# seobbro/TTA-depth-completion

Hardware: AMD Instinct MI355X
Metric: TTA frames/sec (fwd+loss+bwd+Adam) at 352x1216 (higher is better)
Workload: dtype mixed: real frames' forward (the scored depth) f32 storage + bf16x3 MFMA arithmetic; no_grad proxy pass and all data gradients bf16 storage + single bf16 MFMA; fp32 accumulate everywhere; loss / Adam / adapted parameters fp32 (include/ptta.h PTTA_DTYPE_MIXED)

## Files before the change

include/ptta.h:

```cpp
#ifndef PTTA_H
#define PTTA_H
#include <stdint.h>
#ifdef __cplusplus
extern "C" {
#endif

typedef struct ptta_ctx* ptta_handle;
typedef void* ptta_stream;

enum { PTTA_BACKBONE_MSG_CHN = 0, PTTA_BACKBONE_NLSPN = 1, PTTA_BACKBONE_COSTDCNET = 2 };
enum { PTTA_DTYPE_F32 = 0, PTTA_DTYPE_MIXED = 1,
       PTTA_MIXED_KEEP_PROXY = 0x100, PTTA_MIXED_KEEP_BACKWARD = 0x200, PTTA_MIXED_KEEP_HEADS = 0x400,
       PTTA_MIXED_BWD_ROUNDED_W = 0x800 };
enum { PTTA_META_1LAYER = 0, PTTA_META_2LAYERS = 1 };
enum { PTTA_NLSPN_LEGACY_OFFSET = 0x100,
       PTTA_NLSPN_SYNCBN_ADAPT = 0x200,
       PTTA_SYNCBN_ADAPT = 0x200 };

typedef struct {
    float lr, beta1, beta2, eps, weight_decay;
    float w_sparse_depth, w_smoothness, w_cos;
    float max_input_depth;
    float max_predict_depth;
} ptta_hparams;
// ... 46 lines not shown
              const float* validity, float* depth_out, float* loss_info_out, ptta_stream s);

int ptta_outlier_removal(const float* sparse_depth, const float* validity, float* sparse_out, float* validity_out,
                         int n, int height, int width, int kernel_size, float threshold, float* scratch, ptta_stream s);

int ptta_eval_metrics(const float* depth, const float* ground_truth, int64_t numel, float min_evaluate_depth,
                      float max_evaluate_depth, void* scratch, float* metrics_out, ptta_stream s);

int ptta_mdconv_forward(const float* input, const float* weight, const float* bias, const float* offset, const float* mask,
                        float* output, int b, int c, int h, int w, int c_out, int kh, int kw, int sh, int sw, int ph, int pw,
                        int dh, int dw, int group, int deformable_group, ptta_stream s);
int ptta_mdconv_backward(const float* input, const float* weight, const float* bias, const float* offset, const float* mask,
                         const float* grad_output, float* grad_input, float* grad_offset, float* grad_mask, float* grad_weight,
                         float* grad_bias, int b, int c, int h, int w, int c_out, int kh, int kw, int sh, int sw, int ph, int pw,
                         int dh, int dw, int group, int deformable_group, ptta_stream s);

int ptta_set_image_norm(ptta_handle h, float divisor, const float* mean, const float* stdv);

int ptta_head_bind(ptta_handle h, const char* name, float* param, float* exp_avg, float* exp_avg_sq);
int ptta_head_set_hparams(ptta_handle h, float lr, float beta1, float beta2, float eps, float weight_decay, float tau,
                          int adam_step, ptta_stream s);
int ptta_head_reload(ptta_handle h, ptta_stream s);
int ptta_head_forward(ptta_handle h, const float* image, const float* sparse_depth, int reverse, float* emb_out, float* ref_out,
                      ptta_stream s);
int ptta_head_backward(ptta_handle h, float* loss_out, ptta_stream s);
int ptta_head_adam_step(ptta_handle h, ptta_stream s);
int ptta_head_step(ptta_handle h, const float* image, const float* sparse_depth, int reverse, float* loss_out, ptta_stream s);
int ptta_head_get_grad(ptta_handle h, const char* name, float* dst, int64_t capacity, int* has_grad_host, ptta_stream s);

enum { PTTA_HEAD_FORM_PLAIN = 0, PTTA_HEAD_FORM_SYNCBN = 1 };
int ptta_head_set_form(ptta_handle h, int form);

int ptta_crop_flip(const float* src, float* dst, int n, int channels, int height, int width, int crop_height, int crop_width,
                   const int32_t* start_y, const int32_t* start_x, const uint8_t* hflip, const uint8_t* vflip, ptta_stream s);

int ptta_rotate(const float* src, float* dst, int n, int channels, int height, int width, const uint8_t* do_rotate, const float* angle_deg,
                int bilinear, ptta_stream s);
int ptta_resize_crop(const float* src, float* dst, int n, int channels, int height, int width, const uint8_t* do_resize,
                     const int32_t* resize_height, const int32_t* resize_width, const int32_t* start_y, const int32_t* start_x,
                     int bilinear, int scale_depth, ptta_stream s);
int ptta_photometric(const float* src, float* dst, int n, int height, int width, const uint8_t* do_brightness, const float* f_brightness,
                     const uint8_t* do_contrast, const float* f_contrast, const uint8_t* do_saturation, const float* f_saturation,
                     double* scratch, ptta_stream s);

int ptta_photometric_full(const float* src, float* dst, int n, int height, int width, const uint8_t* do_brightness, const float* f_brightness,
                          const uint8_t* do_contrast, const float* f_contrast, const uint8_t* do_gamma, const float* f_gamma,
                          const uint8_t* do_hue, const float* f_hue, const uint8_t* do_saturation, const float* f_saturation,
                          double* scratch, ptta_stream s);
int ptta_add_noise(const float* src, const float* noise, float* dst, int n, int channels, int height, int width, const uint8_t* do_noise,
                   float spread, int uniform, ptta_stream s);
int ptta_remove_patches(const float* src, float* dst, int n, int channels, int height, int width, const uint8_t* do_remove,
                        const uint8_t* selected, const int32_t* patch_height, const int32_t* patch_width, ptta_stream s);
int ptta_crop_pad(const float* src, float* dst, int n, int channels, int height, int width, const uint8_t* do_crop_pad,
                  const int32_t* start_y, const int32_t* start_x, const int32_t* end_y, const int32_t* end_x,
                  const int32_t* pad_top, const int32_t* pad_left, int padding_mode, float fill, ptta_stream s);
int ptta_resize_pad(const float* src, float* dst, int n, int channels, int height, int width, const uint8_t* do_resize_pad,
                    const int32_t* resize_height, const int32_t* resize_width, const int32_t* pad_top, const int32_t* pad_left,
                    int bilinear, int padding_mode, float fill, ptta_stream s);

typedef int (*ptta_allreduce_fn)(void* user, double* exchange_buf, long long count, ptta_stream s);
int ptta_set_stat_sync(ptta_handle h, ptta_allreduce_fn fn, void* user, double* exchange_buf, int64_t capacity, int world_size);

int ptta_rccl_unique_id(void* id128_host);
int ptta_rccl_comm_create(const void* id128_host, int rank, int world_size, void** comm_out_host);
int ptta_rccl_comm_destroy(void* comm);
int ptta_rccl_allreduce_mean_f32(void* comm, float* buf, int64_t count, ptta_stream s);
const char* ptta_rccl_last_error(void);
int ptta_set_stat_sync_rccl(ptta_handle h, void* comm, double* exchange_buf, int64_t capacity, int world_size);
int ptta_set_grad_sync_rccl(ptta_handle h, void* comm);

int ptta_set_graph(ptta_handle h, int enable);

int ptta_set_option(ptta_handle h, const char* key, int value);
int ptta_get_option(ptta_handle h, const char* key, int* value_host);

int ptta_profile(ptta_handle h, int enable);
int ptta_profile_read(ptta_handle h, int klass, double* ms_total_host, double* alg_bytes_host, double* macs_host,
                      int64_t* launches_host, ptta_stream s);

int ptta_debug_tensor(ptta_handle h, const char* name, float* dst, int64_t capacity, int64_t* numel_host, ptta_stream s);
int ptta_op_conv32(const float* in_nhwc, const float* weight, const float* bias, float* out_nhwc,
                   int b, int hin, int win, int mode, int relu_in, int in_major, int flip, int dtype, int naive,
                   ptta_stream s);
int ptta_op_gwgrad(const float* x_nhwc, const float* gy_nhwc, float* gw, float* gb, int b, int h, int w, int ci, int co, int impl,
                   int reps, float* us_per_call_host, ptta_stream s);
#define PTTA_GCONV_S1 0
#define PTTA_GCONV_S2 1
#define PTTA_GCONV_T2 2
#define PTTA_GCONV_VERT 1
#define PTTA_GCONV_X1_W2 2
#define PTTA_GCONV_DGRAD 4
int ptta_op_gconv(const float* x0, int c0, int ld0, const float* x1, int c1, int ld1, const float* weight, const float* bias, float* y,
                  int co, int ldy, int b, int hin, int win, int hout, int wout, int k, int geom, int act, int accumulate, int impl,
                  int flags, int six_b, int x1_from_b, int stat_npass, double* stat_host, int* form_host, ptta_stream s);
#define PTTA_GBN_TRAIN 0
#define PTTA_GBN_EVAL 1
#define PTTA_GBN_BACKWARD 2
typedef struct ptta_gbn_view { float* p; int c; int ld; } ptta_gbn_view;
typedef struct ptta_gbn_args {
    int mode, b, h, w, npass, act, act_first, res_relu, acc_gx, acc_gres, world, nblocks_in, repeats;
    float eps, momentum;
    ptta_gbn_view x, res, y, g, gx, gres;
    const float* gamma; const float* beta; const float* part_in;
    float* st; float* rm; float* rv; long long* nbt; float* st_eval; float* dgamma; float* dbeta;
} ptta_gbn_args;
int ptta_op_gbn(const ptta_gbn_args* a, ptta_stream s);
int ptta_op_conv32_chain(const float* in_nhwc, const float* weight, const float* bias, float* buf_a, float* buf_b, const float* aux,
                         int b, int h, int w, int relu_in, int epi_flags, int reps, int replays, float* us_per_launch_host, ptta_stream s);
#define PTTA_ABI_VERSION 2
int ptta_version(void);

#ifdef __cplusplus
}
#endif
#endif
```

tta-depth-completion_amd/csrc/conv32.hip:

```cpp
#include <cstdlib>
#include <cstring>
#include "ptta_common.h"
#include "ptta_kernels.h"

template <typename T>
struct Conv32P {
    const T* in; int in_nb;
    const void* wpack;
    const void* wpack2;
    Epi<T> epi;
    int B, Hin, Win, Hout, Wout;
};

template <typename T> struct Frag;
template <> struct Frag<float> { typedef float4 A; };
template <> struct Frag<bf16_t> { typedef uint4 A; };

__device__ __forceinline__ float4 relu4(float4 v) {
    v.x = fmaxf(v.x, 0.f); v.y = fmaxf(v.y, 0.f); v.z = fmaxf(v.z, 0.f); v.w = fmaxf(v.w, 0.f);
    return v;
}
__device__ __forceinline__ unsigned relu_bf2(unsigned v) {
    unsigned neg = (v >> 15) & 0x00010001u;
    return v & ~(neg * 0xffffu);
// ... 947 lines not shown
    constexpr int STR = F32 ? S2_STR : 48;
    __shared__ __attribute__((aligned(16))) unsigned char lds[NPIX * STR + WL + 16];
    unsigned char* const wl_lds = lds + NPIX * STR;
    const int tid = threadIdx.x, lane = tid & 63;
    const int i = lane & 31, h = lane >> 5;
    const float biasv = epi_bias(p.epi, i);
    const int wave = __builtin_amdgcn_readfirstlane(tid >> 6);
    const int Hin = p.Hin, Win = p.Win, Ho = p.Hout, Wo = p.Wout;
    const int ntx = (Wo + 31) >> 5, nty = (Ho + S2_TH - 1) / S2_TH;
    const long nstages = 2L * p.B * ntx * nty;
    Px<T> v[NIT];
    auto coords = [&](long tile, int& b, int& oy0, int& ox0) {
        long t_ = tile;
        const int ty = (int)(t_ % nty); t_ /= nty;
        const int tx = (int)(t_ % ntx);
        b = (int)(t_ / ntx); oy0 = ty * S2_TH; ox0 = tx << 5;
    };
    auto issue_loads = [&](long stage) {
        int b, oy0, ox0;
        coords(stage >> 1, b, oy0, ox0);
        const T* inb = p.in + (size_t)(b % p.in_nb) * Hin * Win * 32 + 16 * (int)(stage & 1);
#pragma unroll
        for (int it = 0; it < NIT; ++it) {
            const int idx = tid + 256 * it;
            const int g = idx & 1, pix = idx >> 1;
            const int py = pix / S2_PW, px = pix - py * S2_PW;
            const int gy = 2 * oy0 - 1 + py, gx = 2 * ox0 - 1 + px;
            v[it] = px_zero<T>();
            if (pix < NPIX && gy >= 0 && gy < Hin && gx >= 0 && gx < Win) v[it] = px_load(inb + ((size_t)gy * Win + gx) * 32 + 8 * g);
        }
    };
    const long first = 2L * blockIdx.x, sstride = 2L * gridDim.x;
    if (first < nstages) issue_loads(first);
    uint4 wh[9][2];
    load_weights<T, W2>(wh, wl_lds, p.wpack, p.wpack2, tid, lane);
    f32x16 acc;
    bool started = false;
    for (long base = first; base < nstages; base += sstride) {
        int b, oy0, ox0;
        coords(base >> 1, b, oy0, ox0);
#pragma unroll
        for (int q = 0; q < 2; ++q) {
            if (started) lds_barrier();
            started = true;
#pragma unroll
            for (int it = 0; it < NIT; ++it) {
                const int idx = tid + 256 * it;
                const int pix = idx >> 1;
                if (pix < NPIX) px_stage<RELU>(v[it], lds + pix * STR + 16 * (idx & 1), 32);
            }
            {
                const long nxt = q == 0 ? base + 1 : base + sstride;
                if (nxt < nstages) issue_loads(nxt);
            }
            lds_barrier();
            if (q == 0) {
#pragma unroll
                for (int r = 0; r < 16; ++r) acc[r] = 0.f;
            }
            if (oy0 + wave < Ho) {
#pragma unroll
                for (int tap = 0; tap < 9; ++tap) {
                    const int ky = tap / 3, kx = tap % 3;
                    const unsigned char* a = lds + ((2 * wave + ky) * S2_PW + 2 * i + kx) * STR + 16 * h;
                    const bf16x8 ah = __builtin_bit_cast(bf16x8, *(const uint4*)a);
                    const bf16x8 bh = __builtin_bit_cast(bf16x8, wh[tap][q]);
                    if constexpr (F32) {
                        const bf16x8 al = __builtin_bit_cast(bf16x8, *(const uint4*)(a + 32));
                        const bf16x8 bl = __builtin_bit_cast(bf16x8, *(const uint4*)(wl_lds + ((tap * 2 + q) * 64 + lane) * 16));
                        acc = __builtin_amdgcn_mfma_f32_32x32x16_bf16(al, bh, acc, 0, 0, 0);
                        acc = __builtin_amdgcn_mfma_f32_32x32x16_bf16(ah, bl, acc, 0, 0, 0);
                    } else if constexpr (W2) {
                        const bf16x8 bl = __builtin_bit_cast(bf16x8, *(const uint4*)(wl_lds + ((tap * 2 + q) * 64 + lane) * 16));
                        acc = __builtin_amdgcn_mfma_f32_32x32x16_bf16(ah, bl, acc, 0, 0, 0);
                    }
                    acc = __builtin_amdgcn_mfma_f32_32x32x16_bf16(ah, bh, acc, 0, 0, 0);
                }
                if (q == 1) epi_tile<T, false, MASK, ADD>(p.epi, b, oy0 + wave, Ho, Wo, i, acc, ox0, h, Wo, 1, 0, 0.f, 0.f, nullptr, 0, 0, &biasv);
            }
        }
    }
}

template <typename T, int MODE, bool RELU>
__global__ void conv32_naive_kernel(Conv32P<T> p) {
    const long total = (long)p.B * p.Hout * p.Wout * 32;
    const float* wc = (const float*)p.wpack;
    const float sy = up_scale(p.Hout >> 1, p.Hout), sx = up_scale(p.Wout >> 1, p.Wout);
    for (long idx = (long)blockIdx.x * blockDim.x + threadIdx.x; idx < total; idx += (long)gridDim.x * blockDim.x) {
        const int co = (int)(idx & 31);
        long t_ = idx >> 5;
        const int x = (int)(t_ % p.Wout); t_ /= p.Wout;
        const int y = (int)(t_ % p.Hout);
        const int b = (int)(t_ / p.Hout);
        const T* inb = p.in + (size_t)(b % p.in_nb) * p.Hin * p.Win * 32;
        float acc = 0.f;
        for (int tap = 0; tap < 9; ++tap) {
            const int ky = tap / 3, kx = tap % 3;
            int yi, xi;
            if (MODE == CONV_S1) { yi = y + ky - 1; xi = x + kx - 1; }
            else if (MODE == CONV_S2) { yi = 2 * y + ky - 1; xi = 2 * x + kx - 1; }
            else {
                const int ty = y + 1 - ky, tx = x + 1 - kx;
                if ((ty & 1) || (tx & 1)) continue;
                yi = ty >> 1; xi = tx >> 1;
            }
            if (yi < 0 || yi >= p.Hin || xi < 0 || xi >= p.Win) continue;
            const T* src = inb + ((size_t)yi * p.Win + xi) * 32;
            for (int ci = 0; ci < 32; ++ci) {
                float v = ld(src + ci);
                if (RELU) v = fmaxf(v, 0.f);
                acc = fmaf(v, wc[(tap * 32 + ci) * 32 + co], acc);
            }
        }
        Lerp ly = {0, 0, 0.f, 0.f}, lx = {0, 0, 0.f, 0.f};
        if (p.epi.up) { ly = lerp_coef(y, p.Hout >> 1, sy); lx = lerp_coef(x, p.Wout >> 1, sx); }
        epi_store<T>(p.epi, b, y, x, p.Hout, p.Wout, co, acc, ly, lx);
    }
}

__global__ void pack_conv32_kernel(const float* __restrict__ src, float* mf32, bf16_t* mbf16, bf16_t* mlo, float* canon,
                                   int in_major, int flip, int row_stride, int col_off) {
    const int idx = blockIdx.x * blockDim.x + threadIdx.x;
    if (idx >= 9 * 32 * 32) return;
    const int co = idx & 31, ci = (idx >> 5) & 31, tap = idx >> 10;
    const int st = flip ? 8 - tap : tap;
    const float v = in_major ? src[((size_t)ci * row_stride + col_off + co) * 9 + st] : src[((size_t)co * row_stride + col_off + ci) * 9 + st];
    canon[(tap * 32 + ci) * 32 + co] = v;
    {
        const int g = ci >> 3, hh = (ci >> 2) & 1, s = ci & 3;
        mf32[((tap * 4 + g) * 64 + hh * 32 + co) * 4 + s] = v;
    }
    {
        const int kk = ci >> 4, hh = (ci >> 3) & 1, e = ci & 7;
        const bf16_t hi = f2bf(v);
        mbf16[((tap * 2 + kk) * 64 + hh * 32 + co) * 8 + e] = hi;
        mlo[((tap * 2 + kk) * 64 + hh * 32 + co) * 8 + e] = f2bf(v - bf2f(hi));
    }
}

void ptta_pack_conv32(const float* src, const ConvW& w, int in_major, int flip, hipStream_t s, int row_stride, int col_off) {
    hipLaunchKernelGGL(pack_conv32_kernel, dim3(36), dim3(256), 0, s, src, w.mf32, w.mbf16, w.mlo, w.canon, in_major, flip, row_stride, col_off);
}

template <typename T, int MODE, bool RELU>
static void launch_mfma(const Conv32P<T>& p, int flags, int blocks, hipStream_t s) {
#define K_(U, M, A) hipLaunchKernelGGL((conv32_mfma_kernel<T, MODE, RELU, U, M, A>), dim3(blocks), dim3(256), 0, s, p)
    switch (flags) {
        case 0: K_(false, false, false); break; case 1: K_(true, false, false); break;
        case 2: K_(false, true, false); break;  case 3: K_(true, true, false); break;
        case 4: K_(false, false, true); break;  case 5: K_(true, false, true); break;
        case 6: K_(false, true, true); break;   default: K_(true, true, true); break;
    }
#undef K_
}
template <typename T, bool RELU, bool W2 = false>
static void launch_x3(const Conv32P<T>& p, int flags, int blocks, hipStream_t s) {
    const long tiles8 = (long)p.B * ((p.Wout + 31) / 32) * ((p.Hout + X3_TH - 1) / X3_TH);
    if (tiles8 <= 256) {
        const long t4 = (long)p.B * ((p.Wout + 31) / 32) * ((p.Hout + X3S_TH - 1) / X3S_TH);
        const int nb4 = (int)(t4 > 1024 ? 1024 : t4);
#define KS_(U, M, A) hipLaunchKernelGGL((conv32_s1_small_kernel<T, RELU, U, M, A, W2>), dim3(nb4), dim3(256), 0, s, p)
        switch (flags) {
            case 0: KS_(false, false, false); break; case 1: KS_(true, false, false); break;
            case 2: KS_(false, true, false); break;  case 3: KS_(true, true, false); break;
            case 4: KS_(false, false, true); break;  case 5: KS_(true, false, true); break;
// ... 97 lines not shown
            const long tiles = (long)p.B * ((p.Wout + 31) / 32) * ((p.Hout + S2_TH - 1) / S2_TH);
            const int tb = (int)(tiles < kFullChipBlocks ? tiles : kFullChipBlocks);
#define KS2_(R, M, A) hipLaunchKernelGGL((conv32_s2_lds_kernel<T, R, M, A>), dim3(tb), dim3(256), 0, s, p)
            const bool m_ = flags & 2, a_ = flags & 4;
            if (a.relu_in) { if (m_) { if (a_) KS2_(true, true, true); else KS2_(true, true, false); } else { if (a_) KS2_(true, false, true); else KS2_(true, false, false); } }
            else { if (m_) { if (a_) KS2_(false, true, true); else KS2_(false, true, false); } else { if (a_) KS2_(false, false, true); else KS2_(false, false, false); } }
#undef KS2_
            PTTA_CHECK_LAUNCH();
            return 0;
        }
        if constexpr (MODE != CONV_S1) {
            if (a.relu_in) launch_direct_x3<T, MODE, true>(p, flags, (int)blocks, s); else launch_direct_x3<T, MODE, false>(p, flags, (int)blocks, s);
        }
        PTTA_CHECK_LAUNCH();
        return 0;
    }
    if (a.naive) {
        p.wpack = a.w->canon;
        const long total = (long)p.B * p.Hout * p.Wout * 32;
        int blocks = (int)((total + 255) / 256); if (blocks > 8192) blocks = 8192;
        if (a.relu_in) hipLaunchKernelGGL((conv32_naive_kernel<T, MODE, true>), dim3(blocks), dim3(256), 0, s, p);
        else hipLaunchKernelGGL((conv32_naive_kernel<T, MODE, false>), dim3(blocks), dim3(256), 0, s, p);
    } else {
        if (NAR) return -22;
        p.wpack = (const void*)a.w->mf32;
        const int Wt = (MODE == CONV_T2) ? p.Win : p.Wout;
        const long items = (long)p.B * ((Wt + 31) / 32) * (MODE == CONV_T2 ? 2 : 1) * p.Hout;
        long blocks = (items + 3) / 4;
        if (blocks > 512) blocks = 512;
        if constexpr (!NAR) { if (a.relu_in) launch_mfma<T, MODE, true>(p, flags, (int)blocks, s); else launch_mfma<T, MODE, false>(p, flags, (int)blocks, s); }
    }
    PTTA_CHECK_LAUNCH();
    return 0;
}

template <typename T>
static int launch_first_t(const Conv32Args& a, const ConvInArgs& f, void* a_out, int a_nb, bool bwd_form, long tiles, hipStream_t s) {
    Conv32P<T> p;
    p.in = nullptr; p.in_nb = 1; p.wpack = a.w->mbf16; p.wpack2 = (sizeof(T) == 4 || a.w2) ? a.w->mlo : nullptr;
    p.epi.bias = a.bias; p.epi.up = (const T*)a.up; p.epi.up_nb = a.up_nb > 0 ? a.up_nb : 1;
    p.epi.mask = (const T*)a.mask; p.epi.mask_nb = a.mask_nb > 0 ? a.mask_nb : 1; p.epi.add1 = (const T*)a.add1; p.epi.add1_nb = a.add1_nb > 0 ? a.add1_nb : 1; p.epi.add2 = nullptr; p.epi.add2_nb = 1;
    p.epi.out_raw = (T*)a.out_raw; p.epi.out_sum = (T*)a.out_sum;
    p.epi.mask_bits = a.mask_bits; p.epi.bits_out = a.bits_out; p.epi.bits_nb = a.bits_nb; p.epi.bits_sum = 0;
    p.B = a.B; p.Hin = p.Hout = a.Hin; p.Win = p.Wout = a.Win;
    const int blocks = (int)(tiles > kFullChipBlocks ? kFullChipBlocks : tiles);
    FirstP q;
    for (int c = 0; c < 3; ++c) { q.pl[c] = f.pl[c]; if (q.pl[c].nb < 1) q.pl[c].nb = 1; }
    q.zero_from_b = f.zero_from_b; q.w1 = f.wfrag; q.bias1 = f.bias; q.a_out = (float*)a_out; q.a_nb = a_nb;
    q.fmask_nb = f.mask_nb > 0 ? f.mask_nb : 1; q.fmask_bits = f.mask_bits; q.a_bits = f.a_bits;
    if (bwd_form) {
        if constexpr (sizeof(T) == 2) {
            if (a.w2) {
                if (a.out_sum) hipLaunchKernelGGL((conv32_s1_first_kernel<T, 1, false, true, false, true, true, true>), dim3(blocks), dim3(256), 0, s, p, q);
                else hipLaunchKernelGGL((conv32_s1_first_kernel<T, 1, false, true, false, true, false, true>), dim3(blocks), dim3(256), 0, s, p, q);
                PTTA_CHECK_LAUNCH();
                return 0;
            }
        }
        if (a.out_sum) hipLaunchKernelGGL((conv32_s1_first_kernel<T, 1, false, true, false, true, true>), dim3(blocks), dim3(256), 0, s, p, q);
        else hipLaunchKernelGGL((conv32_s1_first_kernel<T, 1, false, true, false, true>), dim3(blocks), dim3(256), 0, s, p, q);
        PTTA_CHECK_LAUNCH();
        return 0;
    }
#define KF_(C) do { if (a.up) hipLaunchKernelGGL((conv32_s1_first_kernel<T, C, true>), dim3(blocks), dim3(256), 0, s, p, q); \
                    else hipLaunchKernelGGL((conv32_s1_first_kernel<T, C, false>), dim3(blocks), dim3(256), 0, s, p, q); } while (0)
    if (f.cin == 1) KF_(1); else if (f.cin == 2) KF_(2); else KF_(3);
#undef KF_
    PTTA_CHECK_LAUNCH();
    return 0;
}
int ptta_launch_conv32_first(const Conv32Args& a, const ConvInArgs& f, void* a_out, int a_nb, hipStream_t s) {
    const bool bwd_form = f.mask != nullptr;
    if (bwd_form && (!f.mask_bits || !a.mask_bits)) return 1;
    if (a.naive || (!a.bf16 && !a.x3) || a.mode != CONV_S1 || a.add2 || f.naive) return 1;
    if ((a.add1 != nullptr) != (a.out_sum != nullptr) || (a.out_sum && !bwd_form)) return 1;
    if (bwd_form ? (a.relu_in || !a.mask || a.up || f.cin != 1) : (!a.relu_in || a.mask != nullptr)) return 1;
    if (f.cin < 1 || f.cin > 3 || f.up || f.add1 || f.B != a.B || f.H != a.Hin || f.W != a.Win) return 1;
    if (a.bf16 && (a_out || f.a_bits)) return 1;
    const long tiles = (long)a.B * ((a.Win + 31) / 32) * ((a.Hin + X3_TH - 1) / X3_TH);
    if (tiles <= 256) return 1;
    return a.bf16 ? launch_first_t<bf16_t>(a, f, a_out, a_nb, bwd_form, tiles, s) : launch_first_t<float>(a, f, a_out, a_nb, bwd_form, tiles, s);
}

int ptta_launch_conv32(const Conv32Args& a, hipStream_t s) {
    if (a.bf16) {
        if (a.mode == CONV_S1) return launch_conv32_t<bf16_t, CONV_S1>(a, s);
        if (a.mode == CONV_S2) return launch_conv32_t<bf16_t, CONV_S2>(a, s);
        return launch_conv32_t<bf16_t, CONV_T2>(a, s);
    }
    if (a.mode == CONV_S1) return launch_conv32_t<float, CONV_S1>(a, s);
    if (a.mode == CONV_S2) return launch_conv32_t<float, CONV_S2>(a, s);
    return launch_conv32_t<float, CONV_T2>(a, s);
}
```

tta-depth-completion_amd/csrc/msgchn_ctx.h:

```cpp
#pragma once
#include <cstdio>
#include <cstdlib>
#include <cstring>
#include <map>
#include <string>
#include <unordered_map>
#include <vector>

#include "../../include/ptta.h"
#include "ptta_common.h"
#include "ptta_kernels.h"
#include "nlspn.h"

#pragma GCC visibility push(hidden)

#define HIPCHK(x) do { hipError_t e_ = (x); if (e_ != hipSuccess) return c->fail(std::string(#x) + ": " + hipGetErrorString(e_), -100 - (int)e_); } while (0)
#define RUN(x) do { int r_ = (x); if (r_ != 0) return c->fail_chain(std::string(#x) + " failed", r_ < 0 ? r_ : -r_); } while (0)

#define NLFWD(call) do { if (c && c->nl) { c->err.clear(); return (call); } } while (0)

struct ImgNorm { int on; float div; float mean[3]; float stdv[3]; };

namespace msgchn {
hipError_t d2d_copy(void* dst, const void* src, size_t bytes, hipStream_t s);
// ... 11 lines not shown
static constexpr unsigned kStepEvent = hipEventDisableTiming | hipEventDisableSystemFence;
struct L32 { ConvW f{}, b{}; float* bias = nullptr; int transposed = 0; };
struct LIn { float *wfrag = nullptr, *wcanon = nullptr, *bias = nullptr, *bw = nullptr; int cin = 1; };
struct LOut { float *w = nullptr, *bias = nullptr, *bfrag = nullptr, *bcanon = nullptr; };
struct Lin { float *W = nullptr, *Wt = nullptr, *bias = nullptr; bf16_t *Whi = nullptr, *Wlo = nullptr, *Wthi = nullptr, *Wtlo = nullptr, *Wil = nullptr, *Wtil = nullptr;
             bf16_t *Wsl = nullptr, *Wtsl = nullptr;
             int N = 0, K = 0; };
struct BNorm { float *gamma = nullptr, *beta = nullptr, *rm = nullptr, *rv = nullptr; long long* nbt = nullptr;
               float *mean = nullptr, *inv = nullptr, *scale = nullptr, *shift = nullptr; };
struct Dbg { const void* p; long numel; int is_act; };

struct PrefixBufs {
    void *c0 = nullptr, *c1 = nullptr, *c2 = nullptr, *c3 = nullptr, *c4 = nullptr, *e1_0a = nullptr, *e1_0 = nullptr, *e1_1a = nullptr;
    void *c0a = nullptr, *c1a = nullptr, *c2a = nullptr, *c3a = nullptr, *c4a = nullptr;
    void *e1_1 = nullptr, *y1 = nullptr, *e1_2a = nullptr, *y2 = nullptr, *t1 = nullptr, *y3 = nullptr, *s1_1 = nullptr, *u1 = nullptr;
    float *dclamp = nullptr, *d12 = nullptr, *d14 = nullptr, *in_image = nullptr, *in_loss_image = nullptr, *in_sparse = nullptr, *in_validity = nullptr;
    bool proxy_valid = false;
};

struct ptta_ctx : PrefixBufs {
    GNet* nl = nullptr;
    int N = 1, H = 0, W = 0, Hp = 0, Wp = 0, pt = 0, pr = 0, dual = 0, Nn = 1;
    int bf16 = 0, naive = 0, es = 4, x3 = 1;
    int mixed = 0;
    int nar_proxy = 0, nar_bwd = 0, nar_heads = 0;
    std::unordered_map<const void*, void*> ntwin;
    void* tw(const void* p) const { auto it = ntwin.find(p); return it == ntwin.end() ? nullptr : it->second; }
    void twin_alloc(const void* p, int nb, int h, int w) { if (nar_proxy && p) ntwin[p] = dalloc((size_t)nb * h * w * 32 * 2); }
    float *dm_f32 = nullptr;
    ptta_hparams hp{};
    std::string err;
    std::vector<void*> allocs;
    std::map<std::string, L32> l32;
    std::map<std::string, LIn> lin_in;
    std::map<std::string, LOut> lout;
    std::map<std::string, Lin> fc;
    std::map<std::string, BNorm> bn;
    std::map<std::string, Dbg> dbg;
    int meta_mode = 0;
    struct Adapted { std::string name; long n = 0; float *p = nullptr, *m = nullptr, *v = nullptr, *g = nullptr; };
    std::vector<Adapted> adapted;
    struct HeadT { bool ready = false; std::vector<Adapted> prm, tgt; bool has_grad[12] = {};
                   float *hyper = nullptr, *tau2 = nullptr, *loss = nullptr, *loss_part = nullptr, *wpart = nullptr, *bpart = nullptr, *dp = nullptr;
                   float *sv_mean = nullptr, *sv_inv = nullptr, *sv_scale = nullptr, *sv_shift = nullptr;
                   int* step = nullptr; unsigned* ticket = nullptr; PttaAdamEntry *tab = nullptr, *etab = nullptr;
                   std::vector<PttaAdamEntry> tab_host, etab_host; int tab_n = 0; long tab_total = 0, etab_total = 0; int tab_mode = -1; bool etab_dirty = true;
                   int reverse = 1; bool fwd_ok = false, bwd_ok = false;
                   float* garena = nullptr; long garena_n = 0;
                   int form = 0; bool stepped = false; } head;
    int skip_dec3 = 0;
    int head_swap = 0;
    float *meta_w = nullptr, *meta_b = nullptr;
    float *gW = nullptr, *gB = nullptr;
    struct Meta2 {
        ConvW w1f[4], w2f[4], w2b[4];
        void *h[4] = {}, *a1[4] = {}, *t = nullptr, *dt = nullptr, *da1 = nullptr, *dh = nullptr;
        float *st1 = nullptr, *st2 = nullptr;
        float *rm1 = nullptr, *rv1 = nullptr, *rm2 = nullptr, *rv2 = nullptr; long long *nbt1 = nullptr, *nbt2 = nullptr;
        float *cs_part = nullptr, *bw = nullptr;
        bool generic = false;
        float *gh = nullptr, *ga1 = nullptr, *gt = nullptr, *gdt = nullptr, *gda1 = nullptr, *gdh = nullptr;
        float *w1c = nullptr, *w2c = nullptr, *w2bc = nullptr;
        bf16_t *w1hi = nullptr, *w1lo = nullptr, *w2hi = nullptr, *w2lo = nullptr, *w2bhi = nullptr, *w2blo = nullptr;
        float *gst1 = nullptr, *gst2 = nullptr, *part1 = nullptr, *part2 = nullptr, *gbw = nullptr, *gpart = nullptr, *wgp = nullptr;
    } m2;
    float* hyper = nullptr;
    float* w3_tmp = nullptr;
    int* step_dev = nullptr; float* stamp_f = nullptr; unsigned long long* stamp_base = nullptr; int stamps = 0;
    void stamp(int i, hipStream_t s) { if (stamps) msgchn::stamp_launch(stamp_f, stamp_base, i, s); }
    PttaAdamEntry* adam_tab = nullptr; unsigned* adam_ticket = nullptr; bool adam_tab_dirty = true;
    std::vector<PttaAdamEntry> adam_host;
    bool fwd_valid = false;
    PttaStatSync stat_sync;
    Lin fused_pp; bool fused_pp_valid = false; int fuse_heads = 1;
    int heads_v2 = 1;
    int thru = 1; bool thru_active = false;
    int adam_in_wgrad = 1; bool adam_fuse_req = false, adam_fused = false;
    int bwd_w2 = 1;
    const float *cnt_sparse = nullptr, *cnt_validity = nullptr;
    struct { const float *image = nullptr, *sparse = nullptr, *validity = nullptr; bool on = false; } loss_report;
    hipEvent_t ev_loss = nullptr;
    hipEvent_t ev_dpart = nullptr;
    int fuse_first = 1, fuse_head_bwd = 1;
    int cos_grad_fused = 1;
    bool cos_in_gemm = false;
    void* w0frag = nullptr; float *hm_part = nullptr, *headP = nullptr; double* head_k12 = nullptr;
    struct ProfClass { std::vector<std::pair<hipEvent_t, hipEvent_t>> ev; size_t used = 0; double bytes = 0, macs = 0; long launches = 0; };
    bool prof_on = false;
    static constexpr int NPROF = 9;
    ProfClass prof[NPROF];
    std::vector<std::pair<int, size_t>> prof_seq;
    int use_graph = 0;
    void* grad_comm = nullptr;
    float* grad_arena = nullptr; long grad_arena_n = 0;
    int pre_sync_graph = -1, pre_sync_aux = -1;
    hipGraphExec_t gexec[4] = {nullptr, nullptr, nullptr, nullptr};
    hipGraph_t graph[4] = {nullptr, nullptr, nullptr, nullptr};
    hipStream_t cap_stream = nullptr;
    struct PreSet : PrefixBufs {
        bool prepared = false, rest_recorded = false;
        uint64_t prep_token = 0;
        uint64_t last_token = 0;
    };
    PreSet pset[2];
    int cur_set = 0, pipe_cur = 0, pipe_last = 0;
    bool pipe_ready = false, pipe_active = false, skip_prefix = false;
    const float *fb_image = nullptr, *fb_sparse = nullptr;
    hipStream_t pre_stream = nullptr;
    hipEvent_t ev_prefix[2] = {nullptr, nullptr}, ev_rest[2] = {nullptr, nullptr}, ev_entry = nullptr;
    hipStream_t pipe_stream = nullptr; bool pipe_stream_set = false;
    hipGraph_t pgraph[2] = {nullptr, nullptr}, rgraph[4][2] = {{nullptr, nullptr}, {nullptr, nullptr}, {nullptr, nullptr}, {nullptr, nullptr}};
    hipGraphExec_t pexec[2] = {nullptr, nullptr}, rexec[4][2] = {{nullptr, nullptr}, {nullptr, nullptr}, {nullptr, nullptr}, {nullptr, nullptr}};
    int use_aux = 1;
    hipStream_t aux_stream = nullptr;
    hipEvent_t ev_fork = nullptr, ev_join = nullptr, ev_real = nullptr;
    hipEvent_t ev_side[4] = {nullptr, nullptr, nullptr, nullptr};
    hipStream_t aux(hipStream_t caller) {
        if (!use_aux) return nullptr;
        if (!aux_stream) {
            if (hipStreamCreateWithFlags(&aux_stream, hipStreamNonBlocking) != hipSuccess) return nullptr;
            if (hipEventCreateWithFlags(&ev_fork, kStepEvent) != hipSuccess ||
                hipEventCreateWithFlags(&ev_join, kStepEvent) != hipSuccess ||
                hipEventCreateWithFlags(&ev_real, kStepEvent) != hipSuccess ||
                hipEventCreateWithFlags(&ev_side[0], kStepEvent) != hipSuccess || hipEventCreateWithFlags(&ev_side[1], kStepEvent) != hipSuccess ||
                hipEventCreateWithFlags(&ev_side[2], kStepEvent) != hipSuccess || hipEventCreateWithFlags(&ev_side[3], kStepEvent) != hipSuccess) { (void)hipStreamDestroy(aux_stream); aux_stream = nullptr; return nullptr; }
        }
        return prof_on ? caller : aux_stream;
    }
    hipEvent_t ev_replay = nullptr;
    void drop_graphs() {
        if (ev_replay) (void)hipEventSynchronize(ev_replay);
        if (pre_stream) (void)hipStreamSynchronize(pre_stream);
        for (int k = 0; k < 4; ++k) {
            if (gexec[k]) { (void)hipGraphExecDestroy(gexec[k]); gexec[k] = nullptr; }
            if (graph[k]) { (void)hipGraphDestroy(graph[k]); graph[k] = nullptr; }
            for (int p = 0; p < 2; ++p) {
                if (rexec[k][p]) { (void)hipGraphExecDestroy(rexec[k][p]); rexec[k][p] = nullptr; }
                if (rgraph[k][p]) { (void)hipGraphDestroy(rgraph[k][p]); rgraph[k][p] = nullptr; }
            }
        }
        for (int p = 0; p < 2; ++p) {
            if (pexec[p]) { (void)hipGraphExecDestroy(pexec[p]); pexec[p] = nullptr; }
            if (pgraph[p]) { (void)hipGraphDestroy(pgraph[p]); pgraph[p] = nullptr; }
            pset[p].prepared = false; pset[p].prep_token = pset[p].last_token = 0;
        }
        fb_image = fb_sparse = nullptr;
    }

    int err_code = 0;
    int fail(const std::string& m, int code) { err = m; err_code = code; return code; }
    int fail_chain(const std::string& m, int code) { err = (err_code == code && !err.empty() && err.size() < 600) ? m + " <- " + err : m; err_code = code; return code; }

    bool oom = false;
    void* dalloc(size_t bytes) {
        void* p = nullptr;
        if (hipMalloc(&p, bytes ? bytes : 16) != hipSuccess) { oom = true; return nullptr; }
        allocs.push_back(p);
        if (hipMemset(p, 0, bytes ? bytes : 16) != hipSuccess) { oom = true; return nullptr; }
        return p;
    }
    float* falloc(size_t n) { return (float*)dalloc(n * sizeof(float)); }
    void* act(const char* name, int nb, int h, int w) {
        void* p = dalloc((size_t)nb * h * w * 32 * es);
        dbg[name] = Dbg{p, (long)nb * h * w * 32, 1};
        if (nar_proxy && nb == 2 * Nn) twin_alloc(p, Nn, h, w);
        return p;
    }
    void* gact(const char* name, int nb, int h, int w) {
        const int e = nar_bwd ? 2 : es;
        void* p = dalloc((size_t)nb * h * w * 32 * e);
        dbg[name] = Dbg{p, (long)nb * h * w * 32, nar_bwd ? 2 : 1};
        return p;
    }
    int mask_bits_on = 1;
    std::unordered_map<const void*, uint32_t*> mbits;
    void mask_plane(const void* map, int nb, int h, int w) {
        if (bf16 || naive) return;
        if (mbits.count(map)) return;
        mbits[map] = (uint32_t*)dalloc((size_t)nb * h * w * sizeof(uint32_t));
    }
    uint32_t* bits_of(const void* map) const {
        if (!map || !mask_bits_on) return nullptr;
        auto it = mbits.find(map);
        return it == mbits.end() ? nullptr : it->second;
    }
    float* map1(const char* name, int nb, int h, int w) {
        float* p = falloc((size_t)nb * h * w);
        dbg[name] = Dbg{p, (long)nb * h * w, 0};
        return p;
    }

    int H2, W2, H4, W4, H8, W8, H16, W16;
    long Rg = 0;
    float *img_pad = nullptr, *sp_pad = nullptr, *zero_plane = nullptr;
    ImgNorm img_norm = ImgNorm{0, 1.f, {0.f, 0.f, 0.f}, {1.f, 1.f, 1.f}};
    float *out1, *p12, *q, *p11, *depth_net, *depth_final, *validity_tmp;
    void *m, *y4, *s0_1, *v1;
    void *e2_0a, *e2_0, *e2_1a, *e2_1, *e2_2a, *z2, *t2, *z3, *s1_2, *u2, *z4, *s0_2, *v2;
    void *e3_0a, *e3_0, *e3_1a, *e3_1, *e3_2a, *feat, *w2, *t3, *s1_3, *u3, *s0_3, *v3;
    float *h1z, *pz, *h2, *emb, *h1, *ref, *gref_buf, *gmask, *bn_part;
    double* hn_msc = nullptr;
    float* hn_rs = nullptr;
    bool cos_rows_done = false;
    bf16_t *emb_n = nullptr, *ref_n = nullptr, *h2_n = nullptr;
    float *bnb_gscale, *bnb_c1, *bnb_c2;
    float *loss_ws, *loss_info, *g_final, *g_net;
    float* loss_info_dst = nullptr;
    void *dv3, *ds0_3, *du3, *ds1_3, *dt3, *dw2, *dfeat_tot, *dz2_up, *de3_2a, *de3_1, *de3_1a, *de3_0, *de3_0a;
    void *up4_t, *up3_t, *dv2, *ds0_2, *dz4, *du2, *ds1_2, *dz3, *dt2, *dz2, *de2_2a, *de2_1, *de2_1a, *de2_0, *de2_0a, *dv1, *dm_total, *g_feat;
    float *dp11, *dq, *dp12, *dout1, *g_feat_f32;
    float* wgrad_part;
};

struct ProfScope {
    ptta_ctx::ProfClass* pc = nullptr; hipStream_t s;
    ProfScope(ptta_ctx* c, int klass, hipStream_t s_, double bytes, double macs, int launches) : s(s_) {
        if (!c->prof_on) return;
        pc = &c->prof[klass];
        if (pc->used == pc->ev.size()) {
            hipEvent_t e0, e1;
            if (hipEventCreate(&e0) != hipSuccess || hipEventCreate(&e1) != hipSuccess) { pc = nullptr; return; }
            pc->ev.push_back({e0, e1});
        }
        pc->bytes += bytes; pc->macs += macs; pc->launches += launches;
        c->prof_seq.push_back({klass, pc->used});
        (void)hipEventRecord(pc->ev[pc->used].first, s);
    }
    ~ProfScope() { if (pc) { (void)hipEventRecord(pc->ev[pc->used].second, s); pc->used++; } }
};
#define REST_(s_, call) do { ProfScope ps_(c, 8, (s_), 0, 0, 1); RUN(call); } while (0)
#define CV(...) RUN(conv32(c, s, __VA_ARGS__))

struct E { const void* up = nullptr; int up_nb = 1; const void* mask = nullptr; int mask_nb = 1;
           const void* add1 = nullptr; int add1_nb = 1; const void* add2 = nullptr; int add2_nb = 1;
           void* raw = nullptr; void* sum = nullptr;
           bool nar = false; };

inline float* st_ptr(float* base, int C, int pass, int kind) { return base + ((size_t)pass * 4 + kind) * C; }

namespace msgchn {
int pad16(int n);
void build_registry(ptta_ctx* c);
void build_workspace(ptta_ctx* c);
int load_weight(ptta_ctx* c, const std::string& name, const void* tensor, const int64_t* shape, int ndim, hipStream_t s);
int conv_in_p(ptta_ctx* c, const ConvInArgs& a_, hipStream_t s);
int conv_out1_p(ptta_ctx* c, const ConvOut1Args& a, hipStream_t s);
int conv32(ptta_ctx* c, hipStream_t s, const std::string& layer, bool bwd, int mode, const void* in, int in_nb,
           int B, int Hin, int Win, bool relu, const E& e);
int conv32w(ptta_ctx* c, hipStream_t s, const ConvW* w, const float* bias, const void* in, int in_nb, int B, int H, int W, const E& e);
int conv32_first_bwd(ptta_ctx* c, hipStream_t s, const std::string& layer, ConvInArgs& f, int B, int H, int W, const E& e);
int to_narrow(ptta_ctx* c, const void* src_f32, void* dst, long n, hipStream_t s);
int to_wide(ptta_ctx* c, const void* src_nar, float* dst, long n, hipStream_t s);
int rgb_encoder(ptta_ctx* c, const float* image, int nb, int boff, int zero_from_b, hipStream_t s);
int ensure_fused_heads(ptta_ctx* c, hipStream_t s);
int ensure_proxy_rgb(ptta_ctx* c, const float* any_image, hipStream_t s);
int enc1_head_fn(ptta_ctx* c, hipStream_t st);
int stage1_independent(ptta_ctx* c, int B2, hipStream_t s);
bool heads_v2_on(const ptta_ctx* c);
int heads_forward(ptta_ctx* c, hipStream_t s, int part = 0);
int push_hparams(ptta_ctx* c, hipStream_t s);
int forward_common(ptta_ctx* c, const float* image, const float* sparse, bool train, hipStream_t s);
const float* final_depth(ptta_ctx* c);
int heads_backward(ptta_ctx* c, const float* gref, hipStream_t s);
int backbone_backward(ptta_ctx* c, const float* g_net, hipStream_t s, bool join_aux);
void pipe_use(ptta_ctx* c, int p);
void pipe_overwritten(ptta_ctx* c, int p);
int pipe_quiesce(ptta_ctx* c);
int ensure_adam_table(ptta_ctx* c, hipStream_t s);
}
#pragma GCC visibility pop
```

tta-depth-completion_amd/csrc/msgchn_forward.hip:

```cpp
#include "msgchn_ctx.h"

using namespace msgchn;

namespace msgchn {

int conv_in_p(ptta_ctx* c, const ConvInArgs& a_, hipStream_t s) {
    ConvInArgs a = a_;
    const double px = (double)a.B * a.H * a.W;
    ProfScope ps(c, 7, s, px * (a.cin * 4 + 32 * (a.bf16 ? 2 : c->es)) + 9.0 * a.cin * 32 * 4, px * 9.0 * a.cin * 32, 1);
    if (!c->mbits.empty()) {
        if (!a.mask_bits) a.mask_bits = c->bits_of(a.mask);
        if (!a.bf16 && !a.a_bits) { a.a_bits = c->bits_of(a.out_raw); a.a_bits_nb = c->Nn; }
    }
    return ptta_launch_conv_in(a, s);
}
int conv_out1_p(ptta_ctx* c, const ConvOut1Args& a, hipStream_t s) {
    const double px = (double)a.B * a.H * a.W;
    ProfScope ps(c, 7, s, px * (32 * (a.bf16 ? 2 : c->es) + 4) + 288 * 4, px * 288.0, 1);
    return ptta_launch_conv_out1(a, s);
}

int conv32(ptta_ctx* c, hipStream_t s, const std::string& layer, bool bwd, int mode, const void* in, int in_nb,
           int B, int Hin, int Win, bool relu, const E& e) {
    auto it = c->l32.find(layer);
    if (it == c->l32.end()) return c->fail("unknown 32->32 layer " + layer, -2);
    Conv32Args a;
    a.in = in; a.in_nb = in_nb; a.w = bwd ? &it->second.b : &it->second.f;
    a.bias = bwd ? nullptr : (layer == "conv1_rgb_meta" ? c->meta_b : it->second.bias);
    a.up = e.up; a.up_nb = e.up_nb; a.mask = e.mask; a.mask_nb = e.mask_nb;
    a.add1 = e.add1; a.add1_nb = e.add1_nb; a.add2 = e.add2; a.add2_nb = e.add2_nb;
    a.out_raw = e.raw; a.out_sum = e.sum;
    const bool nar = e.nar || (bwd && c->nar_bwd);
    const int es_l = nar ? 2 : c->es;
    a.B = B; a.Hin = Hin; a.Win = Win; a.mode = mode; a.relu_in = relu ? 1 : 0; a.bf16 = nar ? 1 : c->bf16; a.naive = c->naive; a.x3 = c->x3;
    a.w2 = (bwd && c->nar_bwd && c->bwd_w2) ? 1 : 0;
    if (!c->mbits.empty()) {
        a.mask_bits = c->bits_of(e.mask);
        if (!bwd && !nar) {
            uint32_t* bs = c->bits_of(e.sum); uint32_t* br = c->bits_of(e.raw);
            if (bs && br) return c->fail("conv32: both outputs of " + layer + " are registered masks", -22);
            if (bs || br) { a.bits_out = bs ? bs : br; a.bits_sum = bs ? 1 : 0; a.bits_nb = c->Nn; }
        }
    }
    const long pin = (long)B * Hin * Win;
    const long pout = mode == CONV_S1 ? pin : (mode == CONV_S2 ? pin / 4 : pin * 4);
    const bool small = (long)Hin * Win <= (long)c->H4 * c->W4 * (mode == CONV_S2 ? 4 : 1);
#ifdef PTTA_EXP_SKIP_PAIRED_S1
    if (mode == CONV_S1 && small && layer.size() > 2 && layer.compare(layer.size() - 2, 2, ".3") == 0 && layer.find("prdct") == std::string::npos) return 0;
#endif
    ProfScope ps(c, (mode == CONV_S1 ? (relu ? 0 : 2) : 4) + (small ? 1 : 0), s, (double)((pin + pout) * 32 + 9216) * es_l,
                 (double)(mode == CONV_T2 ? pin : pout) * 9.0 * 32.0 * 32.0, 1);
    return ptta_launch_conv32(a, s);
}

int conv32w(ptta_ctx* c, hipStream_t s, const ConvW* w, const float* bias, const void* in, int in_nb, int B, int H, int W, const E& e) {
    Conv32Args a;
    a.in = in; a.in_nb = in_nb; a.w = w; a.bias = bias;
    a.add1 = e.add1; a.add1_nb = e.add1_nb; a.out_raw = e.raw; a.out_sum = e.sum;
    a.B = B; a.Hin = H; a.Win = W; a.mode = CONV_S1; a.relu_in = 0; a.bf16 = c->bf16; a.naive = c->naive; a.x3 = c->x3;
    return ptta_launch_conv32(a, s);
}

static int conv32_first(ptta_ctx* c, hipStream_t s, const std::string& layer, ConvInArgs& f, int a_nb, int B, int H, int W, const E& e) {
    auto it = c->l32.find(layer);
    if (it == c->l32.end()) return c->fail("unknown 32->32 layer " + layer, -2);
    const long tiles = (long)B * ((W + 31) / 32) * ((H + 7) / 8);
    const bool nar = e.nar;
    f.bf16 = nar ? 1 : c->bf16;
    if (c->fuse_first >= (f.cin == 3 ? 2 : 1) && !c->bf16 && !c->naive && c->x3 && tiles > 256 && !e.mask && !e.add1 && !e.add2 && !e.sum) {
        Conv32Args a;
        a.in = nullptr; a.in_nb = B; a.w = &it->second.f; a.bias = it->second.bias;
        a.up = e.up; a.up_nb = e.up_nb; a.out_raw = e.raw;
        a.B = B; a.Hin = H; a.Win = W; a.mode = CONV_S1; a.relu_in = 1; a.bf16 = nar ? 1 : 0; a.naive = 0; a.x3 = 1;
        const double px = (double)B * H * W;
        const int es_l = nar ? 2 : c->es;
        ProfScope ps(c, 0, s, (px * f.cin + 9.0 * f.cin * 32) * 4 + (px * 96 + 9216) * es_l, px * 9.0 * (f.cin * 32 + 1024), 1);
        f.a_bits = (a_nb > 0 && !nar) ? c->bits_of(f.out_raw) : nullptr;
        if (!c->mbits.empty() && !nar) { uint32_t* br = c->bits_of(e.raw); if (br) { a.bits_out = br; a.bits_nb = c->Nn; } }
        const int rc = ptta_launch_conv32_first(a, f, (a_nb > 0 && !nar && !f.a_bits) ? f.out_raw : nullptr, a_nb, s);
        return rc == 1 ? c->fail("conv32_first: fused form refused a case its caller accepted", -22) : rc;
    }
    RUN(conv_in_p(c, f, s));
    return conv32(c, s, layer, false, CONV_S1, f.out_raw, B, B, H, W, true, e);
}

int conv32_first_bwd(ptta_ctx* c, hipStream_t s, const std::string& layer, ConvInArgs& f, int B, int H, int W, const E& e) {
    auto it = c->l32.find(layer);
    if (it == c->l32.end()) return c->fail("unknown 32->32 layer " + layer, -2);
    const long tiles = (long)B * ((W + 31) / 32) * ((H + 7) / 8);
    const bool nar = c->nar_bwd != 0;
    f.bf16 = nar ? 1 : c->bf16;
    if (c->fuse_head_bwd && c->bits_of(f.mask) && c->bits_of(e.mask) && c->fuse_first >= 1 && !c->bf16 && !c->naive && c->x3 && tiles > 256 && e.mask && e.raw && (e.add1 != nullptr) == (e.sum != nullptr) && !e.add2 && !e.up) {
        Conv32Args a;
        a.in = nullptr; a.in_nb = B; a.w = &it->second.b; a.bias = nullptr;
        a.mask = e.mask; a.mask_nb = e.mask_nb; a.out_raw = e.raw; a.add1 = e.add1; a.add1_nb = e.add1_nb; a.out_sum = e.sum;
        a.mask_bits = c->bits_of(e.mask); f.mask_bits = c->bits_of(f.mask);
        a.B = B; a.Hin = H; a.Win = W; a.mode = CONV_S1; a.relu_in = 0; a.bf16 = nar ? 1 : 0; a.naive = 0; a.x3 = 1;
        a.w2 = (nar && c->bwd_w2) ? 1 : 0;
        const double px = (double)B * H * W;
        const int es_l = nar ? 2 : c->es;
        ProfScope ps(c, 2, s, (px + 9.0 * 32) * 4 + (px * 96 + 9216) * es_l, px * 9.0 * (32 + 1024), 1);
        const int rc = ptta_launch_conv32_first(a, f, nullptr, 0, s);
        return rc == 1 ? c->fail("conv32_first_bwd: fused form refused a case its caller accepted", -22) : rc;
    }
    RUN(conv_in_p(c, f, s));
    return conv32(c, s, layer, true, CONV_S1, f.out_raw, B, B, H, W, false, e);
}


static int meta_forward(ptta_ctx* c, bool train, int B, hipStream_t s) {
    const int H4 = c->H4, W4 = c->W4, Nn = c->Nn;
    if (c->meta_mode == PTTA_META_1LAYER) {
        E e; e.raw = c->m;
        if (c->nar_proxy && train && B == 2 * Nn) {
            return conv32(c, s, "conv1_rgb_meta", false, CONV_S1, c->c2, Nn, Nn, H4, W4, false, e);
        }
        return conv32(c, s, "conv1_rgb_meta", false, CONV_S1, c->c2, B, B, H4, W4, false, e);
    }
    auto& m2 = c->m2;
    const ptta_ctx::Adapted* A = c->adapted.data();
    const long P = (long)Nn * H4 * W4;
    const int npass = train ? B / Nn : 1;
    if (m2.generic) {
        if (!train && (!m2.rm1 || !m2.rv1 || !m2.rm2 || !m2.rv2)) return c->fail("meta BatchNorm running statistics not loaded", -3);
        GView x; x.p = (float*)c->c2; x.B = B; x.H = H4; x.W = W4; x.C = 32; x.ld = 32;
        GView hv = x; hv.p = m2.gh; hv.C = 128; hv.ld = 128;
        GView av = hv; av.p = m2.ga1;
        GView tv = x; tv.p = m2.gt;
        GView mv = x; mv.p = (float*)c->m;
        const int tiles_pp = ptta_gconv_x3_tiles(B / npass, H4, W4);
        auto finalize = [&](float* part, int C, const float* gamma, const float* beta, float* rm, float* rv, long long* nbt, float* st) -> int {
            if (!train) return ptta_launch_bn_eval_affine(gamma, beta, rm, rv, 1e-5f, st + 2 * C, st + 3 * C, C, s);
            if (ptta_stat_sync(&c->stat_sync, part, tiles_pp, C, npass, s)) return -5;
            const int wmul = c->stat_sync.world > 1 ? c->stat_sync.world : 1;
            for (int pass = 0; pass < npass; ++pass)
// ... 17 lines not shown
        RUN(ptta_launch_gconv_x3(b2, 3, s));
        RUN(finalize(m2.part2, 32, A[5].p, A[6].p, m2.rm2, m2.rv2, m2.nbt2, m2.gst2));
        RUN(ptta_launch_gbn_apply(tv, x, mv, npass, GACT_NONE, m2.gst2, 0, s));
        return 0;
    }
    const int nblk = ptta_chan_stats_blocks();
    for (int g = 0; g < 4; ++g) { E e; e.raw = m2.h[g]; RUN(conv32w(c, s, &m2.w1f[g], nullptr, c->c2, B, B, H4, W4, e)); }
    if (train) {
        for (int pass = 0; pass < npass; ++pass)
            for (int g = 0; g < 4; ++g) {
                RUN(ptta_launch_chan_stats32(m2.h[g], nullptr, c->bf16, pass * P, P, nullptr, nullptr, nullptr, nullptr, -1.f, m2.cs_part, s));
                RUN(ptta_launch_bn_finalize(m2.cs_part, nblk, (int)P, 32, A[1].p + 32 * g, A[2].p + 32 * g, 1e-5f, 0.1f,
                                            m2.rm1 ? m2.rm1 + 32 * g : nullptr, m2.rv1 ? m2.rv1 + 32 * g : nullptr, g == 0 ? m2.nbt1 : nullptr,
                                            st_ptr(m2.st1, 128, pass, 0) + 32 * g, st_ptr(m2.st1, 128, pass, 1) + 32 * g,
                                            st_ptr(m2.st1, 128, pass, 2) + 32 * g, st_ptr(m2.st1, 128, pass, 3) + 32 * g, s));
            }
    } else {
        if (!m2.rm1 || !m2.rv1 || !m2.rm2 || !m2.rv2) return c->fail("meta BatchNorm running statistics not loaded", -3);
        RUN(ptta_launch_bn_eval_affine(A[1].p, A[2].p, m2.rm1, m2.rv1, 1e-5f, st_ptr(m2.st1, 128, 0, 2), st_ptr(m2.st1, 128, 0, 3), 128, s));
    }
    for (int g = 0; g < 4; ++g)
        RUN(ptta_launch_bn_apply32(m2.h[g], nullptr, m2.a1[g], c->bf16, (long)B * H4 * W4, train ? P : (long)B * H4 * W4,
                                   st_ptr(m2.st1, 128, 0, 2) + 32 * g, st_ptr(m2.st1, 128, 0, 3) + 32 * g, 4 * 128, 0.2f, s));
    for (int g = 0; g < 4; ++g) {
        E e;
        if (g == 0) e.raw = m2.t; else { e.add1 = m2.t; e.add1_nb = B; e.sum = m2.t; }
        RUN(conv32w(c, s, &m2.w2f[g], g == 0 ? A[4].p : nullptr, m2.a1[g], B, B, H4, W4, e));
    }
    if (train) {
        for (int pass = 0; pass < npass; ++pass) {
            RUN(ptta_launch_chan_stats32(m2.t, nullptr, c->bf16, pass * P, P, nullptr, nullptr, nullptr, nullptr, -1.f, m2.cs_part, s));
            RUN(ptta_launch_bn_finalize(m2.cs_part, nblk, (int)P, 32, A[5].p, A[6].p, 1e-5f, 0.1f, m2.rm2, m2.rv2, m2.nbt2,
                                        st_ptr(m2.st2, 32, pass, 0), st_ptr(m2.st2, 32, pass, 1), st_ptr(m2.st2, 32, pass, 2), st_ptr(m2.st2, 32, pass, 3), s));
        }
    } else {
        RUN(ptta_launch_bn_eval_affine(A[5].p, A[6].p, m2.rm2, m2.rv2, 1e-5f, st_ptr(m2.st2, 32, 0, 2), st_ptr(m2.st2, 32, 0, 3), 32, s));
    }
    RUN(ptta_launch_bn_apply32(m2.t, c->c2, c->m, c->bf16, (long)B * H4 * W4, train ? P : (long)B * H4 * W4,
                               st_ptr(m2.st2, 32, 0, 2), st_ptr(m2.st2, 32, 0, 3), 4 * 32, -1.f, s));
    return 0;
}


int to_narrow(ptta_ctx* c, const void* src_f32, void* dst, long n, hipStream_t s) {
    if (!src_f32 || !dst) return c->fail("to_narrow: missing narrow twin", -22);
    ProfScope ps_(c, 8, s, 0, 0, 1);
    from_f32_launch((const float*)src_f32, (bf16_t*)dst, n, s);
    return 0;
}
int to_wide(ptta_ctx* c, const void* src_nar, float* dst, long n, hipStream_t s) {
    if (!src_nar || !dst) return c->fail("to_wide: missing operand", -22);
    ProfScope ps_(c, 8, s, 0, 0, 1);
    to_f32_launch((const bf16_t*)src_nar, dst, n, s);
    return 0;
}
static int meta_forward_proxy(ptta_ctx* c, hipStream_t s) {
    const int H4 = c->H4, W4 = c->W4, Nn = c->Nn;
    const long half = (long)Nn * H4 * W4 * 32;
    if (c->meta_mode == PTTA_META_1LAYER) {
        E e; e.raw = c->tw(c->m); e.nar = true;
        return conv32(c, s, "conv1_rgb_meta", false, CONV_S1, c->tw(c->c2), Nn, Nn, H4, W4, false, e);
    }
    return to_narrow(c, (const float*)c->m + half, c->tw(c->m), half, s);
}


int rgb_encoder(ptta_ctx* c, const float* image, int nb, int boff, int zero_from_b, hipStream_t s) {
    const int H1 = c->Hp, W1 = c->Wp, H2 = c->H2, W2 = c->W2, H4 = c->H4, W4 = c->W4, H8 = c->H8, W8 = c->W8, H16 = c->H16, W16 = c->W16;
    auto at = [&](void* base, int h, int w) { return (void*)((char*)base + (size_t)boff * h * w * 32 * c->es); };
    auto e_raw = [](void* raw) { E e; e.raw = raw; return e; };
    {
        const LIn& li = c->lin_in["rgb_encoder.init.0"];
        ConvInArgs a; a.cin = 3; a.zero_from_b = zero_from_b;
        for (int ch = 0; ch < 3; ++ch) {
            a.pl[ch].p = image + (size_t)ch * H1 * W1; a.pl[ch].nb = c->Nn; a.pl[ch].bstride = 3L * H1 * W1;
            if (c->img_norm.on && !c->dual) {
                a.pl[ch].norm = 1; a.pl[ch].div = c->img_norm.div; a.pl[ch].mean = c->img_norm.mean[ch]; a.pl[ch].stdv = c->img_norm.stdv[ch];
            }
        }
        a.wfrag = li.wfrag; a.wcanon = li.wcanon; a.bias = li.bias; a.out_raw = at(c->c0a, H1, W1);
        a.B = nb; a.H = H1; a.W = W1; a.bf16 = c->bf16; a.naive = c->naive;
        RUN(conv32_first(c, s, "rgb_encoder.init.2", a, 0, nb, H1, W1, e_raw(at(c->c0, H1, W1))));
    }
    CV("rgb_encoder.enc1.1", false, CONV_S2, at(c->c0, H1, W1), nb, nb, H1, W1, true, e_raw(at(c->c1a, H2, W2)));
    CV("rgb_encoder.enc1.3", false, CONV_S1, at(c->c1a, H2, W2), nb, nb, H2, W2, true, e_raw(at(c->c1, H2, W2)));
    CV("rgb_encoder.enc2.1", false, CONV_S2, at(c->c1, H2, W2), nb, nb, H2, W2, true, e_raw(at(c->c2a, H4, W4)));
    CV("rgb_encoder.enc2.3", false, CONV_S1, at(c->c2a, H4, W4), nb, nb, H4, W4, true, e_raw(at(c->c2, H4, W4)));
    CV("rgb_encoder.enc3.1", false, CONV_S2, at(c->c2, H4, W4), nb, nb, H4, W4, true, e_raw(at(c->c3a, H8, W8)));
    CV("rgb_encoder.enc3.3", false, CONV_S1, at(c->c3a, H8, W8), nb, nb, H8, W8, true, e_raw(at(c->c3, H8, W8)));
    CV("rgb_encoder.enc4.1", false, CONV_S2, at(c->c3, H8, W8), nb, nb, H8, W8, true, e_raw(at(c->c4a, H16, W16)));
    CV("rgb_encoder.enc4.3", false, CONV_S1, at(c->c4a, H16, W16), nb, nb, H16, W16, true, e_raw(at(c->c4, H16, W16)));
    return 0;
}

int ensure_fused_heads(ptta_ctx* c, hipStream_t s) {
    if (c->fused_pp_valid || !c->fuse_heads) return 0;
    Lin& f = c->fused_pp; const Lin& a = c->fc["proj.3"]; const Lin& b = c->fc["pred.0"];
    fuse_linear_launch(b.W, b.bias, a.W, a.bias, f.W, f.bias, 512, 512, 512, s);
    ptta_split_weight(f.W, f.Whi, f.Wlo, f.Wil, 512L * 512, 512, s);
    ptta_hn_pack_w(f.Whi, f.Wsl, 512, s);
    c->fused_pp_valid = true;
    return 0;
}

int ensure_proxy_rgb(ptta_ctx* c, const float* any_image, hipStream_t s) {
    RUN(ensure_fused_heads(c, s));
    if (c->proxy_valid) return 0;
    RUN(rgb_encoder(c, any_image, c->Nn, c->Nn, 0, s));
    if (c->nar_proxy) {
        const int Nn = c->Nn;
        struct { void* p; int h, w; } maps[4] = {{c->c1, c->H2, c->W2}, {c->c2, c->H4, c->W4}, {c->c3, c->H8, c->W8}, {c->c4, c->H16, c->W16}};
        for (auto& m_ : maps) {
            const long half = (long)Nn * m_.h * m_.w * 32;
            RUN(to_narrow(c, (const float*)m_.p + half, c->tw(m_.p), half, s));
        }
    }
    c->proxy_valid = true;
    return 0;
}

int enc1_head_fn(ptta_ctx* c, hipStream_t st) {
    const int Nn = c->Nn, H4 = c->H4, W4 = c->W4;
    const LIn& li = c->lin_in["depth_encoder1.init.0"];
    ConvInArgs a; a.cin = 1; a.pl[0].p = c->d14; a.pl[0].nb = Nn; a.pl[0].bstride = (long)H4 * W4;
    a.wfrag = li.wfrag; a.wcanon = li.wcanon; a.bias = li.bias; a.out_raw = c->e1_0a;
    a.B = Nn; a.H = H4; a.W = W4; a.bf16 = c->bf16; a.naive = c->naive;
    RUN(conv_in_p(c, a, st));
    { E e; e.raw = c->e1_0; RUN(conv32(c, st, "depth_encoder1.init.2", false, CONV_S1, c->e1_0a, Nn, Nn, H4, W4, true, e)); }
    { E e; e.raw = c->e1_1a; RUN(conv32(c, st, "depth_encoder1.enc1.1", false, CONV_S2, c->e1_0, Nn, Nn, H4, W4, true, e)); }
    return 0;
}

int stage1_independent(ptta_ctx* c, int B2, hipStream_t s) {
    const int Nn = c->Nn, H4 = c->H4, W4 = c->W4, H8 = c->H8, W8 = c->W8, H16 = c->H16, W16 = c->W16;
    const bool two = c->nar_proxy && B2 == 2 * Nn;
    const int Bf = two ? Nn : B2;
    { E e; e.raw = c->e1_1; e.sum = c->y1; e.add1 = c->c3; e.add1_nb = B2;
      RUN(conv32(c, s, "depth_encoder1.enc1.3", false, CONV_S1, c->e1_1a, Nn, Bf, H8, W8, true, e)); }
    { E e; e.raw = c->e1_2a; RUN(conv32(c, s, "depth_encoder1.enc2.1", false, CONV_S2, c->e1_1, B2, Nn, H8, W8, true, e)); }
    { E e; e.sum = c->y2; e.add1 = c->c4; e.add1_nb = B2;
      RUN(conv32(c, s, "depth_encoder1.enc2.3", false, CONV_S1, c->e1_2a, Nn, Bf, H16, W16, true, e)); }
    { E e; e.raw = c->t1; RUN(conv32(c, s, "depth_decoder1.dec2.1", false, CONV_T2, c->y2, B2, Bf, H16, W16, true, e)); }
    { E e; e.raw = c->y3; e.sum = c->s1_1; e.add1 = c->y1; e.add1_nb = B2;
      RUN(conv32(c, s, "depth_decoder1.dec2.3", false, CONV_S1, c->t1, B2, Bf, H8, W8, true, e)); }
    { E e; e.raw = c->u1; RUN(conv32(c, s, "depth_decoder1.dec1.1", false, CONV_T2, c->s1_1, B2, Bf, H8, W8, true, e)); }
    if (!two) return 0;
    RUN(to_narrow(c, c->e1_0, c->tw(c->e1_0), (long)Nn * H4 * W4 * 32, s));
    RUN(to_narrow(c, c->e1_1a, c->tw(c->e1_1a), (long)Nn * H8 * W8 * 32, s));
    RUN(to_narrow(c, c->e1_2a, c->tw(c->e1_2a), (long)Nn * H16 * W16 * 32, s));
    { E e; e.nar = true; e.sum = c->tw(c->y1); e.add1 = c->tw(c->c3); e.add1_nb = Nn;
      RUN(conv32(c, s, "depth_encoder1.enc1.3", false, CONV_S1, c->tw(c->e1_1a), Nn, Nn, H8, W8, true, e)); }
    { E e; e.nar = true; e.sum = c->tw(c->y2); e.add1 = c->tw(c->c4); e.add1_nb = Nn;
      RUN(conv32(c, s, "depth_encoder1.enc2.3", false, CONV_S1, c->tw(c->e1_2a), Nn, Nn, H16, W16, true, e)); }
    { E e; e.nar = true; e.raw = c->tw(c->t1); RUN(conv32(c, s, "depth_decoder1.dec2.1", false, CONV_T2, c->tw(c->y2), Nn, Nn, H16, W16, true, e)); }
    { E e; e.nar = true; e.raw = c->tw(c->y3); e.sum = c->tw(c->s1_1); e.add1 = c->tw(c->y1); e.add1_nb = Nn;
      RUN(conv32(c, s, "depth_decoder1.dec2.3", false, CONV_S1, c->tw(c->t1), Nn, Nn, H8, W8, true, e)); }
    { E e; e.nar = true; e.raw = c->tw(c->u1); RUN(conv32(c, s, "depth_decoder1.dec1.1", false, CONV_T2, c->tw(c->s1_1), Nn, Nn, H8, W8, true, e)); }
    return 0;
}

static int backbone(ptta_ctx* c, const float* image, bool train, hipStream_t s) {
    hipStream_t s2 = train ? c->aux(s) : nullptr;
    const int Nn = c->Nn, B2 = train ? 2 * Nn : Nn;
    const bool two = train && c->nar_proxy;
    const int H1 = c->Hp, W1 = c->Wp, H2 = c->H2, W2 = c->W2, H4 = c->H4, W4 = c->W4, H8 = c->H8, W8 = c->W8, H16 = c->H16, W16 = c->W16;
    auto e_raw = [](void* raw) { E e; e.raw = raw; return e; };
    if (!c->skip_prefix) RUN(rgb_encoder(c, image, Nn, 0, Nn, s));
    RUN(meta_forward(c, train, B2, s));
    if (!c->skip_prefix) { RUN(enc1_head_fn(c, s)); RUN(stage1_independent(c, B2, s)); }

    auto region = [&](hipStream_t st, int b0, int Bl, bool nar) -> int {
        auto A = [&](void* p_, int h, int w) -> void* { return nar ? c->tw(p_) : (void*)((char*)p_ + (size_t)b0 * h * w * 32 * c->es); };
        auto P1 = [&](float* p_, int h, int w) { return p_ + (size_t)b0 * h * w; };
        auto raw = [&](void* r) { E e; e.raw = r; e.nar = nar; return e; };
        const void* e1_0 = nar ? c->tw(c->e1_0) : c->e1_0;
#define CR(...) RUN(conv32(c, st, __VA_ARGS__))
        { E e; e.nar = nar; e.raw = A(c->y4, H4, W4); e.sum = A(c->s0_1, H4, W4); e.add1 = e1_0; e.add1_nb = Nn; e.add2 = A(c->m, H4, W4); e.add2_nb = Bl;
          CR("depth_decoder1.dec1.3", false, CONV_S1, A(c->u1, H4, W4), Bl, Bl, H4, W4, true, e); }
        CR("depth_decoder1.prdct.1", false, CONV_S1, A(c->s0_1, H4, W4), Bl, Bl, H4, W4, true, raw(A(c->v1, H4, W4)));
        {
            const LOut& lo = c->lout["depth_decoder1.prdct.3"];
            ConvOut1Args a; a.in = A(c->v1, H4, W4); a.in_nb = Bl; a.w = lo.w; a.bias = lo.bias; a.out = P1(c->out1, H4, W4);
            a.B = Bl; a.H = H4; a.W = W4; a.relu_in = 1; a.bf16 = nar ? 1 : c->bf16;
            RUN(conv_out1_p(c, a, st));
        }
        REST_(st, ptta_launch_up2_1ch(P1(c->out1, H4, W4), P1(c->p12, H2, W2), Bl, H4, W4, st));
        {
            const LIn& li = c->lin_in["depth_encoder2.init.0"];
            ConvInArgs a; a.cin = 2;
            a.pl[0].p = c->d12; a.pl[0].nb = Nn; a.pl[0].bstride = (long)H2 * W2;
            a.pl[1].p = P1(c->p12, H2, W2); a.pl[1].nb = Bl; a.pl[1].bstride = (long)H2 * W2;
            a.wfrag = li.wfrag; a.wcanon = li.wcanon; a.bias = li.bias; a.out_raw = A(c->e2_0a, H2, W2);
            a.B = Bl; a.H = H2; a.W = W2; a.bf16 = c->bf16; a.naive = c->naive;
            E e; e.nar = nar; e.raw = A(c->e2_0, H2, W2); e.up = A(c->y4, H4, W4); e.up_nb = Bl;
            RUN(conv32_first(c, st, "depth_encoder2.init.2", a, (b0 == 0 && !nar) ? Nn : 0, Bl, H2, W2, e));
        }
        CR("depth_encoder2.enc1.1", false, CONV_S2, A(c->e2_0, H2, W2), Bl, Bl, H2, W2, true, raw(A(c->e2_1a, H4, W4)));
        { E e; e.nar = nar; e.raw = A(c->e2_1, H4, W4); e.up = A(c->y3, H8, W8); e.up_nb = Bl; CR("depth_encoder2.enc1.3", false, CONV_S1, A(c->e2_1a, H4, W4), Bl, Bl, H4, W4, true, e); }
        CR("depth_encoder2.enc2.1", false, CONV_S2, A(c->e2_1, H4, W4), Bl, Bl, H4, W4, true, raw(A(c->e2_2a, H8, W8)));
        { E e; e.nar = nar; e.sum = A(c->z2, H8, W8); e.up = A(c->y2, H16, W16); e.up_nb = Bl; e.add1 = A(c->c3, H8, W8); e.add1_nb = Bl;
          CR("depth_encoder2.enc2.3", false, CONV_S1, A(c->e2_2a, H8, W8), Bl, Bl, H8, W8, true, e); }
        CR("depth_decoder2.dec2.1", false, CONV_T2, A(c->z2, H8, W8), Bl, Bl, H8, W8, true, raw(A(c->t2, H4, W4)));
        { E e; e.nar = nar; e.raw = A(c->z3, H4, W4); e.sum = A(c->s1_2, H4, W4); e.add1 = A(c->e2_1, H4, W4); e.add1_nb = Bl; e.add2 = A(c->m, H4, W4); e.add2_nb = Bl;
          CR("depth_decoder2.dec2.3", false, CONV_S1, A(c->t2, H4, W4), Bl, Bl, H4, W4, true, e); }
        CR("depth_decoder2.dec1.1", false, CONV_T2, A(c->s1_2, H4, W4), Bl, Bl, H4, W4, true, raw(A(c->u2, H2, W2)));
        { E e; e.nar = nar; e.raw = A(c->z4, H2, W2); e.sum = A(c->s0_2, H2, W2); e.add1 = A(c->e2_0, H2, W2); e.add1_nb = Bl; e.add2 = A(c->c1, H2, W2); e.add2_nb = Bl;
          CR("depth_decoder2.dec1.3", false, CONV_S1, A(c->u2, H2, W2), Bl, Bl, H2, W2, true, e); }
        CR("depth_decoder2.prdct.1", false, CONV_S1, A(c->s0_2, H2, W2), Bl, Bl, H2, W2, true, raw(A(c->v2, H2, W2)));
        {
            const LOut& lo = c->lout["depth_decoder2.prdct.3"];
            ConvOut1Args a; a.in = A(c->v2, H2, W2); a.in_nb = Bl; a.w = lo.w; a.bias = lo.bias; a.add = P1(c->p12, H2, W2); a.add_nb = Bl; a.out = P1(c->q, H2, W2);
            a.B = Bl; a.H = H2; a.W = W2; a.relu_in = 1; a.bf16 = nar ? 1 : c->bf16;
            RUN(conv_out1_p(c, a, st));
        }
        REST_(st, ptta_launch_up2_1ch(P1(c->q, H2, W2), P1(c->p11, H1, W1), Bl, H2, W2, st));
        {
            const LIn& li = c->lin_in["depth_encoder3.init.0"];
            ConvInArgs a; a.cin = 2;
            a.pl[0].p = c->dclamp; a.pl[0].nb = Nn; a.pl[0].bstride = (long)H1 * W1;
            a.pl[1].p = P1(c->p11, H1, W1); a.pl[1].nb = Bl; a.pl[1].bstride = (long)H1 * W1;
            a.wfrag = li.wfrag; a.wcanon = li.wcanon; a.bias = li.bias; a.out_raw = A(c->e3_0a, H1, W1);
            a.B = Bl; a.H = H1; a.W = W1; a.bf16 = c->bf16; a.naive = c->naive;
            E e; e.nar = nar; e.raw = A(c->e3_0, H1, W1); e.up = A(c->z4, H2, W2); e.up_nb = Bl;
            RUN(conv32_first(c, st, "depth_encoder3.init.2", a, (b0 == 0 && !nar) ? Nn : 0, Bl, H1, W1, e));
        }
        CR("depth_encoder3.enc1.1", false, CONV_S2, A(c->e3_0, H1, W1), Bl, Bl, H1, W1, true, raw(A(c->e3_1a, H2, W2)));
        { E e; e.nar = nar; e.raw = A(c->e3_1, H2, W2); e.up = A(c->z3, H4, W4); e.up_nb = Bl; CR("depth_encoder3.enc1.3", false, CONV_S1, A(c->e3_1a, H2, W2), Bl, Bl, H2, W2, true, e); }
        CR("depth_encoder3.enc2.1", false, CONV_S2, A(c->e3_1, H2, W2), Bl, Bl, H2, W2, true, raw(A(c->e3_2a, H4, W4)));
        { E e; e.nar = nar; e.raw = A(c->feat, H4, W4); e.up = A(c->z2, H8, W8); e.up_nb = Bl; e.add1 = A(c->m, H4, W4); e.add1_nb = Bl;
          if (!nar) e.sum = A(c->w2, H4, W4); else e.add1 = nullptr;
          CR("depth_encoder3.enc2.3", false, CONV_S1, A(c->e3_2a, H4, W4), Bl, Bl, H4, W4, true, e); }
#undef CR
        return 0;
    };
    if (two) {
        hipStream_t sp = s2 ? s2 : s;
        if (s2) { HIPCHK(hipEventRecord(c->ev_fork, s)); HIPCHK(hipStreamWaitEvent(s2, c->ev_fork, 0)); }
        c->stamp(3, sp);
        if (s2 && c->thru_active && c->cnt_sparse) REST_(s2, ptta_launch_loss_valid_count(c->cnt_sparse, c->cnt_validity, c->N, c->H, c->W, c->loss_ws, s2));
        RUN(meta_forward_proxy(c, sp));
        c->stamp(1, s);
        RUN(region(s, 0, Nn, false));
        c->stamp(2, s);
        RUN(region(sp, Nn, Nn, true));
        c->stamp(4, sp);
        const bool hn = c->nar_heads && heads_v2_on(c);
        if (!hn) RUN(to_wide(c, c->tw(c->feat), (float*)c->feat + (size_t)c->Rg * 32, c->Rg * 32, sp));
        if (s2) {
            if (hn) RUN(heads_forward(c, s2, 1));
            c->stamp(5, s2);
            HIPCHK(hipEventRecord(c->ev_real, s)); HIPCHK(hipStreamWaitEvent(s2, c->ev_real, 0));
            RUN(heads_forward(c, s2, hn ? 2 : 0));
            c->stamp(6, s2);
            HIPCHK(hipEventRecord(c->ev_join, s2));
        }
    } else {
        RUN(region(s, 0, B2, false));
        if (train && s2) {
            HIPCHK(hipEventRecord(c->ev_fork, s)); HIPCHK(hipStreamWaitEvent(s2, c->ev_fork, 0));
            if (c->thru_active && c->cnt_sparse) REST_(s2, ptta_launch_loss_valid_count(c->cnt_sparse, c->cnt_validity, c->N, c->H, c->W, c->loss_ws, s2));
            RUN(heads_forward(c, s2));
            HIPCHK(hipEventRecord(c->ev_join, s2));
        }
    }
    if (!c->skip_dec3) {
    CV("depth_decoder3.dec2.1", false, CONV_T2, c->w2, B2, Nn, H4, W4, true, e_raw(c->t3));
    { E e; e.sum = c->s1_3; e.add1 = c->e3_1; e.add1_nb = B2; e.add2 = c->c1; e.add2_nb = B2;
      CV("depth_decoder3.dec2.3", false, CONV_S1, c->t3, Nn, Nn, H2, W2, true, e); }
    CV("depth_decoder3.dec1.1", false, CONV_T2, c->s1_3, Nn, Nn, H2, W2, true, e_raw(c->u3));
    { E e; e.sum = c->s0_3; e.add1 = c->e3_0; e.add1_nb = B2; e.add2 = c->c0; e.add2_nb = B2;
      CV("depth_decoder3.dec1.3", false, CONV_S1, c->u3, Nn, Nn, H1, W1, true, e); }
    CV("depth_decoder3.prdct.1", false, CONV_S1, c->s0_3, Nn, Nn, H1, W1, true, e_raw(c->v3));
    {
        const LOut& lo = c->lout["depth_decoder3.prdct.3"];
        ConvOut1Args a; a.in = c->v3; a.in_nb = Nn; a.w = lo.w; a.bias = lo.bias; a.add = c->p11; a.add_nb = B2; a.out = c->depth_net;
        a.B = Nn; a.H = H1; a.W = W1; a.relu_in = 1; a.bf16 = c->bf16;
        RUN(conv_out1_p(c, a, s));
    }
    }
    c->stamp(7, s);
    if (train) {
        if (s2) { if (!c->thru_active) HIPCHK(hipStreamWaitEvent(s, c->ev_join, 0)); }
        else RUN(heads_forward(c, s));
    }
    return 0;
}

bool heads_v2_on(const ptta_ctx* c) {
    return c->heads_v2 && c->fuse_heads && c->fused_pp_valid && c->x3 && !c->bf16 && !c->naive && !c->skip_dec3 && !c->head_swap;
}

static int mlp_forward(ptta_ctx* c, const std::string& name, const void* A, int a_bf16, int K, float* hidden, float* out, hipStream_t s) {
    const Lin& l0 = c->fc[name + ".0"]; const Lin& l3 = c->fc[name + ".3"]; BNorm& bn = c->bn[name + ".1"];
    const int R = (int)c->Rg;
    GemmArgs g; g.A = A; g.a_bf16 = a_bf16; g.W = l0.W; g.bias = l0.bias; g.C = hidden; g.R = R; g.K = K; g.N = 512; g.epi = 1; g.part = c->bn_part;
    g.x3 = c->x3; g.Whi = l0.Whi; g.Wlo = l0.Wlo; g.Wil = l0.Wil;
    RUN(ptta_launch_gemm(g, s));
    RUN(ptta_stat_sync(&c->stat_sync, c->bn_part, ptta_gemm_part_blocks(g), 512, 1, s));
    RUN(ptta_launch_bn_finalize(c->bn_part, ptta_gemm_part_blocks(g), R * (c->stat_sync.world > 1 ? c->stat_sync.world : 1), 512, bn.gamma, bn.beta, 1e-5f, 0.1f, bn.rm, bn.rv, bn.nbt,
                                bn.mean, bn.inv, bn.scale, bn.shift, s));
    GemmArgs g2; g2.A = hidden; g2.W = l3.W; g2.bias = l3.bias; g2.C = out; g2.R = R; g2.K = 512; g2.N = 512; g2.pro = 1;
    g2.pscale = bn.scale; g2.pshift = bn.shift;
    g2.x3 = c->x3; g2.Whi = l3.Whi; g2.Wlo = l3.Wlo; g2.Wil = l3.Wil;
    RUN(ptta_launch_gemm(g2, s));
    return 0;
}

int heads_forward(ptta_ctx* c, hipStream_t s, int part) {
    if (part != 1) c->cos_rows_done = false;
    const double esh = (c->nar_heads && heads_v2_on(c)) ? 2.0 : 4.0;
    ProfScope ps_(c, 6, s, (double)c->Rg * 2 * 32 * 4 + ((double)c->Rg * (2 * 512 + 4 * 1024) + 2 * 16384.0 + 4 * 262144.0) * esh,
                  (double)c->Rg * (2 * 16384.0 + 4 * 262144.0), heads_v2_on(c) ? 7 : 8);
    const size_t half = (size_t)c->Rg * 32 * c->es;
    const void* feat_zero = (const char*)c->feat + half;
    if (c->nar_heads && heads_v2_on(c)) {
        const Lin& l0 = c->fc["proj.0"]; const Lin& lf = c->fused_pp; const Lin& lp3 = c->fc["pred.3"]; const Lin& l3 = c->fc["proj.3"];
        BNorm& b1 = c->bn["proj.1"]; BNorm& b2 = c->bn["pred.1"];
        const long R = c->Rg; const int Rw = (int)R * (c->stat_sync.world > 1 ? c->stat_sync.world : 1);
        const int nbh = 2, nb = ptta_hn_row_blocks(R);
        float* part_real = c->hm_part; float* part_zero = c->hm_part + (size_t)nbh * 2 * 512;
        double* msc_real = c->hn_msc; double* msc_zero = c->hn_msc + (size_t)ptta_hn_moment_scratch(R);
        HnBnOut bo1; bo1.gamma = b1.gamma; bo1.beta = b1.beta; bo1.rm = b1.rm; bo1.rv = b1.rv; bo1.nbt = b1.nbt;
        bo1.mean = b1.mean; bo1.inv = b1.inv; bo1.scale = b1.scale; bo1.shift = b1.shift;
        auto gemm_h = [&](const void* x, int x_bf16, const Lin& w, bf16_t* out, int epi) {
            HnGemmArgs g; g.pro = 3; g.epi = epi; g.X = x; g.x_bf16 = x_bf16; g.W0 = l0.Whi; g.b0 = l0.bias; g.pscale = b1.scale; g.pshift = b1.shift;
            g.W = w.Wsl; g.bias = w.bias; g.C = out; g.part = c->bn_part; g.R = R;
            return g;
        };
        if (part != 2) {
            const void* xz = c->nar_proxy ? (const void*)c->tw(c->feat) : (const void*)((const float*)c->feat + (size_t)R * 32);
            if (!c->stat_sync.on()) RUN(ptta_launch_hn_moments(xz, c->nar_proxy ? 1 : 0, R, 1, l0.W, l0.bias, msc_zero, nullptr, &bo1, s));
            else {
            RUN(ptta_launch_hn_moments(xz, c->nar_proxy ? 1 : 0, R, 1, l0.W, l0.bias, msc_zero, part_zero, nullptr, s));
            RUN(ptta_stat_sync(&c->stat_sync, part_zero, nbh, 512, 1, s));
            RUN(ptta_launch_bn_finalize(part_zero, nbh, Rw, 512, b1.gamma, b1.beta, 1e-5f, 0.1f, b1.rm, b1.rv, b1.nbt, b1.mean, b1.inv, b1.scale, b1.shift, s));
            }
            if (c->nar_proxy) RUN(ptta_launch_hn_gemm(gemm_h(c->tw(c->feat), 1, lf, c->h2_n, 1), s));
            else RUN(ptta_launch_hn_gemm(gemm_h((const float*)c->feat + (size_t)R * 32, 0, lf, c->h2_n, 1), s));
            RUN(ptta_stat_sync(&c->stat_sync, c->bn_part, nb, 512, 1, s));
            RUN(ptta_launch_bn_finalize(c->bn_part, nb, Rw, 512, b2.gamma, b2.beta, 1e-5f, 0.1f, b2.rm, b2.rv, b2.nbt, b2.mean, b2.inv, b2.scale, b2.shift, s));
            HnGemmArgs g3; g3.pro = 1; g3.epi = 2; g3.A = c->h2_n; g3.pscale = b2.scale; g3.pshift = b2.shift; g3.W = lp3.Wsl; g3.bias = lp3.bias; g3.C = c->emb_n; g3.R = R;
            g3.rs = c->hn_rs;
            RUN(ptta_launch_hn_gemm(g3, s));
        }
        if (part != 1) {
            if (!c->stat_sync.on()) RUN(ptta_launch_hn_moments(c->feat, 0, R, 1, l0.W, l0.bias, msc_real, nullptr, &bo1, s));
            else {
            RUN(ptta_launch_hn_moments(c->feat, 0, R, 1, l0.W, l0.bias, msc_real, part_real, nullptr, s));
            RUN(ptta_stat_sync(&c->stat_sync, part_real, nbh, 512, 1, s));
            RUN(ptta_launch_bn_finalize(part_real, nbh, Rw, 512, b1.gamma, b1.beta, 1e-5f, 0.1f, b1.rm, b1.rv, b1.nbt, b1.mean, b1.inv, b1.scale, b1.shift, s));
            }
            HnGemmArgs gr = gemm_h(c->feat, 0, l3, c->ref_n, 5);
            gr.E = c->emb_n; gr.rs = c->hn_rs; gr.rowstats_out = c->loss_ws + ptta_loss_ws_rows_off(c->N);
            gr.cpart = c->loss_ws + ptta_loss_ws_cos_off(c->N, c->Rg); gr.cpart_n = ptta_loss_cos_blocks(c->Rg);
// ... 131 lines not shown
```

tta-depth-completion_amd/csrc/ptta_api.hip:

```cpp
#include "msgchn_ctx.h"

using namespace msgchn;

int msgchn::ensure_adam_table(ptta_ctx* c, hipStream_t s) {
    if (!c->adam_tab_dirty) return 0;
    for (auto& ad : c->adapted) if (!ad.p || !ad.m || !ad.v) return 0;
    c->adam_host.resize(c->adapted.size());
    long off = 0;
    for (size_t k = 0; k < c->adapted.size(); ++k) { auto& ad = c->adapted[k]; c->adam_host[k] = PttaAdamEntry{ad.p, ad.m, ad.v, ad.g, ad.n, off}; off += ad.n; }
    HIPCHK(hipMemcpyAsync(c->adam_tab, c->adam_host.data(), c->adam_host.size() * sizeof(PttaAdamEntry), hipMemcpyHostToDevice, s));
    c->adam_tab_dirty = false;
    return 0;
}

extern "C" {

int ptta_version(void) { return PTTA_ABI_VERSION; }

const char* ptta_last_error(ptta_handle h) { return h ? (h->nl && h->err.empty() ? h->nl->err.c_str() : h->err.c_str()) : "null handle"; }

static int wrap_gnet(ptta_handle* out, GNet* e, int rc, int gmix, int n, int height, int width, const ptta_hparams* hp) {
    if (!e) return rc ? rc : -12;
    e->mixed = e->naive ? 0 : gmix;
    ptta_ctx* c = new ptta_ctx();
// ... 280 lines not shown
int ptta_adam_step(ptta_handle c, const float* gw, const float* gb, ptta_stream s_) {
    if (c && c->nl) return (gw || gb) ? c->fail("explicit gradients are an MSG_CHN 1layer convenience", -22) : c->nl->adam_step((hipStream_t)s_);

    if (!c) return -1;
    for (auto& ad : c->adapted) if (!ad.p || !ad.m || !ad.v) return c->fail("Adam state of " + ad.name + " not bound", -3);
    if ((gw || gb) && c->meta_mode != PTTA_META_1LAYER) return c->fail("explicit gradients are a 1layer convenience; use the internal ones", -22);
    hipStream_t s = (hipStream_t)s_;
    if (!gw && !gb) {
        RUN(ensure_adam_table(c, s));
        long total = 0; for (auto& ad : c->adapted) total += ad.n;
        REST_(s, ptta_launch_adam_multi(c->adam_tab, (int)c->adapted.size(), total, c->hyper, c->step_dev, c->adam_ticket, s));
        return 0;
    }
    RUN(ptta_launch_step_inc(c->step_dev, s));
    for (size_t k = 0; k < c->adapted.size(); ++k) {
        auto& ad = c->adapted[k];
        const float* g = ad.g;
        if (c->meta_mode == PTTA_META_1LAYER) { if (k == 0 && gw) g = gw; if (k == 1 && gb) g = gb; }
        RUN(ptta_launch_adam(ad.p, ad.m, ad.v, g, ad.n, c->hyper, c->step_dev, s));
    }
    return 0;
}

int ptta_set_image_norm(ptta_handle c, float divisor, const float* mean, const float* stdv) {
    NLFWD(c->nl->set_image_norm(divisor, mean, stdv));

    if (!c) return -1;
    if (!(divisor > 0.f)) return c->fail("ptta_set_image_norm: divisor must be positive", -22);
    ImgNorm nm = ImgNorm{0, divisor, {0.f, 0.f, 0.f}, {1.f, 1.f, 1.f}};
    for (int k = 0; k < 3; ++k) {
        if (mean) nm.mean[k] = mean[k];
        if (stdv) { if (!(stdv[k] > 0.f)) return c->fail("ptta_set_image_norm: std must be positive", -22); nm.stdv[k] = stdv[k]; }
    }
    nm.on = !(divisor == 1.f && nm.mean[0] == 0.f && nm.mean[1] == 0.f && nm.mean[2] == 0.f && nm.stdv[0] == 1.f &&
              nm.stdv[1] == 1.f && nm.stdv[2] == 1.f);
    c->img_norm = nm;
    c->drop_graphs();
    return 0;
}

static int set_stat_sync(ptta_ctx* c, const PttaStatSync& sy, bool on, bool keeps_graph) {
    if (c->nl) { c->err.clear(); c->nl->drop_graphs(); c->nl->stat_sync = sy; return 0; }
    if (on && c->meta_mode == PTTA_META_2LAYERS && !c->m2.generic) return c->fail("SyncBatchNorm needs the default arithmetic for the 2layers meta layer", -38);
    c->stat_sync = sy;
    c->drop_graphs();
    if (on) {
        if (c->pre_sync_graph < 0) { c->pre_sync_graph = c->use_graph; c->pre_sync_aux = c->use_aux; }
        else if (keeps_graph) c->use_graph = c->pre_sync_graph;
        if (!keeps_graph) c->use_graph = 0;
        c->use_aux = 0;
    } else if (c->pre_sync_graph >= 0) {
        c->use_graph = c->pre_sync_graph; c->use_aux = c->pre_sync_aux; c->pre_sync_graph = c->pre_sync_aux = -1;
    }
    return 0;
}

int ptta_set_stat_sync(ptta_handle c, ptta_allreduce_fn fn, void* user, double* exchange_buf, int64_t capacity, int world_size) {
    if (!c || world_size < 1 || (world_size > 1 && (!fn || !exchange_buf || capacity < 2 * 1024))) return -22;
    PttaStatSync sy; sy.fn = (ptta_allreduce_cb)fn; sy.user = user; sy.buf = exchange_buf; sy.cap = (long)capacity; sy.world = world_size;
    return set_stat_sync(c, sy, world_size > 1, false);
}

int ptta_set_stat_sync_rccl(ptta_handle c, void* comm, double* exchange_buf, int64_t capacity, int world_size) {
    if (!c || world_size < 1 || (comm && (!exchange_buf || capacity < 2 * 1024))) return -22;
    PttaStatSync sy; sy.comm = comm; sy.buf = exchange_buf; sy.cap = (long)capacity; sy.world = world_size;
    return set_stat_sync(c, sy, comm != nullptr, true);
}

int ptta_set_grad_sync_rccl(ptta_handle c, void* comm) {
    if (!c) return -1;
    if (c->nl) { c->nl->drop_graphs(); c->nl->grad_comm = comm; return 0; }
    c->grad_comm = comm;
    c->drop_graphs();
    return 0;
}

struct Option { const char* key; int ptta_ctx::*member; int hi; bool mixed_free; };
static const Option kOptions[] = {
    {"aux_stream", &ptta_ctx::use_aux, 1, true},        {"thru", &ptta_ctx::thru, 1, true},
    {"adam_in_wgrad", &ptta_ctx::adam_in_wgrad, 1, true}, {"bwd_w2", &ptta_ctx::bwd_w2, 1, true},
    {"fuse_first", &ptta_ctx::fuse_first, 2, false},    {"fuse_head_bwd", &ptta_ctx::fuse_head_bwd, 1, false},
    {"fuse_heads", &ptta_ctx::fuse_heads, 1, false},    {"heads_v2", &ptta_ctx::heads_v2, 1, false},
    {"cos_in_gemm", &ptta_ctx::cos_grad_fused, 1, false}, {"mask_bits", &ptta_ctx::mask_bits_on, 1, false},
    {"stamps", &ptta_ctx::stamps, 1, true},
};
static const Option* find_option(const std::string& k) {
    for (const Option& o : kOptions) if (k == o.key) return &o;
    return nullptr;
}
int ptta_set_option(ptta_handle c, const char* key, int value) {
    if (!c || !key) return -1;
    const std::string k(key);
    if (k == "graph") return ptta_set_graph(c, value);
    if (c->nl) return -38;
    const Option* o = find_option(k);
    if (!o) return c->fail("ptta_set_option: unknown key '" + k + "'", -22);
    int* f = &(c->*(o->member));
    if (value < 0 || value > o->hi) return c->fail("ptta_set_option: value out of range for '" + k + "'", -22);
    if (c->mixed && !o->mixed_free && value != 1)
        return c->fail("ptta_set_option: the mixed mode is defined on the default kernels ('" + k + "' stays 1)", -38);
    if (k == "aux_stream" && c->pre_sync_graph >= 0) { c->pre_sync_aux = value; return 0; }
    if (*f == value) return 0;
    RUN(pipe_quiesce(c));
    c->drop_graphs();
    *f = value;
    return 0;
}

int ptta_get_option(ptta_handle c, const char* key, int* value) {
    if (!c || !key || !value) return -1;
    const std::string k(key);
    if (k == "pipelined_active") { *value = !(c->nl || c->prof_on || c->dual || c->stat_sync.on() || c->grad_comm || c->naive || c->bf16); return 0; }
    if (k == "thru_active") { *value = c->nl ? 0 : (c->thru && c->cos_grad_fused && heads_v2_on(c) && c->use_aux); return 0; }
    if (c->nl) { if (k != "graph") return -38; *value = c->nl->use_graph; return 0; }
    if (k == "graph") { *value = c->use_graph; return 0; }
    const Option* o = find_option(k);
    if (!o) return -22;
    *value = c->*(o->member);
    return 0;
}

int ptta_set_graph(ptta_handle c, int enable) {
    if (c && c->nl) { c->nl->use_graph = enable ? 1 : 0; if (!enable) c->nl->drop_graphs(); return 0; }

    if (!c) return -1;
    if (enable && c->stat_sync.on() && !c->stat_sync.comm) return c->fail("graph replay is not available with SyncBatchNorm exchange (ptta_set_stat_sync)", -38);
    c->use_graph = enable ? 1 : 0;
    if (!enable) c->drop_graphs();
    return 0;
}

int ptta_profile(ptta_handle c, int enable) {
    if (c && c->nl) return c->fail("not available for the NLSPN / CostDCNet backbones: use ptta_step / ptta_forward_*", -38);

    if (!c) return -1;
    c->prof_on = enable != 0;
    for (auto& pc : c->prof) { pc.used = 0; pc.bytes = 0; pc.macs = 0; pc.launches = 0; }
    c->prof_seq.clear();
    return 0;
}

int ptta_profile_read(ptta_handle c, int klass, double* ms_total, double* alg_bytes, double* macs, int64_t* launches, ptta_stream s_) {
    if (c && c->nl) return c->fail("not available for the NLSPN / CostDCNet backbones: use ptta_step / ptta_forward_*", -38);

    if (!c || klass < 0 || klass >= ptta_ctx::NPROF) return -1;
    HIPCHK(hipStreamSynchronize((hipStream_t)s_));
    ptta_ctx::ProfClass& pc = c->prof[klass];
    double ms = 0;
    for (size_t k = 0; k < pc.used; ++k) {
        float t = 0.f;
        HIPCHK(hipEventElapsedTime(&t, pc.ev[k].first, pc.ev[k].second));
        ms += t;
    }
    if (ms_total) *ms_total = ms;
    if (alg_bytes) *alg_bytes = pc.bytes;
    if (macs) *macs = pc.macs;
    if (launches) *launches = (int64_t)pc.launches;
    return 0;
}

int ptta_debug_tensor(ptta_handle c, const char* name, float* dst, int64_t capacity, int64_t* numel_host, ptta_stream s_) {
    NLFWD(c->nl->debug_tensor(name, dst, capacity, numel_host, (hipStream_t)s_));

    if (!c || !name) return -1;
    if (std::string(name) == "prof_seq") {
        HIPCHK(hipStreamSynchronize((hipStream_t)s_));
        const int64_t n = 2 * (int64_t)c->prof_seq.size();
// ... 28 lines not shown
```

tta-depth-completion_amd/csrc/ptta_kernels.h:

```cpp
#pragma once
#include <hip/hip_runtime.h>
#include <cstdlib>
#include <cstring>
#include "ptta_common.h"

struct PttaCreateEnv { int naive = 0, exact = 0, graph = -1; };
inline PttaCreateEnv ptta_create_env() {
    PttaCreateEnv e;
    const char* v = getenv("PTTA_CONV_IMPL"); e.naive = (v && strcmp(v, "naive") == 0) ? 1 : 0;
    v = getenv("PTTA_ARITH"); e.exact = (v && strcmp(v, "exact") == 0) ? 1 : 0;
    v = getenv("PTTA_GRAPH"); e.graph = (v && (strcmp(v, "0") == 0 || strcmp(v, "1") == 0)) ? (v[0] - '0') : -1;
    return e;
}

struct ConvW {
    float* mf32;
    bf16_t* mbf16;
    bf16_t* mlo;
    float* canon;
};
struct Conv32Args {
    const void* in = nullptr; int in_nb = 1;
    const ConvW* w = nullptr;
    const float* bias = nullptr;
    const void* up = nullptr; int up_nb = 1;
    const void* mask = nullptr; int mask_nb = 1;
    const void* add1 = nullptr; int add1_nb = 1;
    const void* add2 = nullptr; int add2_nb = 1;
    void* out_raw = nullptr; void* out_sum = nullptr;
    int B = 1, Hin = 0, Win = 0;
    int mode = CONV_S1; int relu_in = 0; int bf16 = 0; int naive = 0;
    int x3 = 0;
    int w2 = 0;
    const uint32_t* mask_bits = nullptr;
    uint32_t* bits_out = nullptr; int bits_nb = 0; int bits_sum = 0;
};
void ptta_pack_conv32(const float* src, const ConvW& w, int in_major, int flip, hipStream_t s, int row_stride = 32, int col_off = 0);
int ptta_launch_conv32(const Conv32Args& a, hipStream_t s);
int ptta_launch_conv32_loop(const Conv32Args& a, void* buf_a, void* buf_b, int reps, unsigned* ctr, unsigned* base_io, int* err, int variant, hipStream_t s);

struct Plane { const float* p = nullptr; int nb = 1; long bstride = 0;
               int norm = 0; float div = 1.f, mean = 0.f, stdv = 1.f; };
struct ConvInArgs {
    Plane pl[3]; int cin = 1; int zero_from_b = 1 << 30;
    const float* wfrag = nullptr;
    const float* wcanon = nullptr;
    const float* bias = nullptr;
    const void* up = nullptr; int up_nb = 1;
    const void* mask = nullptr; int mask_nb = 1;
    const void* add1 = nullptr; int add1_nb = 1;
    void* out_raw = nullptr; void* out_sum = nullptr;
    int B = 1, H = 0, W = 0; int bf16 = 0; int naive = 0;
    const uint32_t* mask_bits = nullptr; uint32_t* a_bits = nullptr;
    int a_bits_nb = 0;
};
void ptta_pack_conv_in(const float* src, int cin_total, int cin_first, int cin, int transpose_flip,
                       float* wfrag, float* wcanon, hipStream_t s);
int ptta_launch_conv_in(const ConvInArgs& a, hipStream_t s);
int ptta_launch_conv32_first(const Conv32Args& a, const ConvInArgs& f, void* a_out, int a_nb, hipStream_t s);

struct ConvOut1Args {
    const void* in = nullptr; int in_nb = 1;
    const float* w = nullptr;
    const float* bias = nullptr;
    const float* add = nullptr; int add_nb = 1;
    float* out = nullptr;
    int B = 1, H = 0, W = 0; int relu_in = 0; int bf16 = 0;
};
void ptta_pack_conv_out1(const float* src, int src_cin_total, int src_cin_index, int from_conv_in, float* w, hipStream_t s);
int ptta_launch_conv_out1(const ConvOut1Args& a, hipStream_t s);

int ptta_launch_prep(const float* sparse, float max_input_depth, float* dclamp, float* d12, float* d14,
                     int N, int H, int W, hipStream_t s);
int ptta_launch_up2_1ch(const float* in, float* out, int B, int Hin, int Win, hipStream_t s);
int ptta_launch_up2T_1ch(const float* gout, float* gin, int B, int Hin, int Win, hipStream_t s);
int ptta_launch_up2T_32(const void* gout, const void* add, void* gin, int B, int Hin, int Win, int bf16, hipStream_t s);

int ptta_launch_outlier_removal(const float* sparse, const float* validity, float* sparse_out, float* validity_out,
                                int N, int H, int W, int ksize, float threshold, float* scratch, hipStream_t s);

typedef int (*ptta_allreduce_cb)(void* user, double* dev_buf, long long count, void* stream);
int ptta_rccl_sum_f64(void* comm, double* buf, long long count, hipStream_t s);
struct PttaStatSync {
    ptta_allreduce_cb fn = nullptr; void* user = nullptr;
    void* comm = nullptr;
    double* buf = nullptr; long cap = 0; int world = 1;
    bool on() const { return (fn || comm) && (world > 1 || comm); }
    int exchange(long long count, hipStream_t s) const {
        if (comm) return ptta_rccl_sum_f64(comm, buf, count, s);
        const int rc = fn(user, buf, count, (void*)s);
        return rc ? (rc < 0 ? rc : -rc) : 0;
    }
};
int ptta_stat_sync(const PttaStatSync* sy, float* part, int nblocks, int C, int npass, hipStream_t s);
int ptta_grad_mean_sync(const PttaStatSync* sy, float* g, long n, hipStream_t s);

struct GemmArgs {
    const void* A = nullptr; int a_bf16 = 0;
    const float* A2 = nullptr;
    const float* W = nullptr;
    const float* bias = nullptr;
    float* C = nullptr;
    int R = 0, K = 0, N = 0;
    int pro = 0;
    const float* pscale = nullptr; const float* pshift = nullptr;
    const float* pmean = nullptr; const float* pinv = nullptr;
    const float* pc1 = nullptr; const float* pc2 = nullptr;
    int epi = 0;
    const float* eH = nullptr;
    const float* escale = nullptr; const float* eshift = nullptr; const float* emean = nullptr; const float* einv = nullptr;
    float* part = nullptr;
    int x3 = 0; const bf16_t* Whi = nullptr; const bf16_t* Wlo = nullptr;
    const bf16_t* Wil = nullptr;
    const float* X = nullptr;
    const void* W0frag = nullptr;
    const float* b0 = nullptr;
    const bf16_t* W0hi = nullptr; const bf16_t* W0lo = nullptr;
    const bf16_t* W0thi = nullptr; const bf16_t* W0tlo = nullptr;
    float* P = nullptr;
    const float* Bref = nullptr; const float* rowstats = nullptr; const float* coef = nullptr;
};
// ... 195 lines not shown
```

tta-depth-completion_amd/csrc/ptta_ops.hip:

```cpp
#include "msgchn_ctx.h"
#include "gnet.h"

using namespace msgchn;

namespace {
struct ScratchConvW {
    ConvW w{};
    bool ok;
    ScratchConvW() {
        ok = hipMalloc((void**)&w.mf32, 9 * 4 * 64 * 4 * 4) == hipSuccess && hipMalloc((void**)&w.mbf16, 9 * 2 * 64 * 8 * 2) == hipSuccess &&
             hipMalloc((void**)&w.canon, 9216 * 4) == hipSuccess && hipMalloc((void**)&w.mlo, 9 * 2 * 64 * 8 * 2) == hipSuccess;
    }
    ~ScratchConvW() { (void)hipFree(w.mf32); (void)hipFree(w.mbf16); (void)hipFree(w.mlo); (void)hipFree(w.canon); }
    ScratchConvW(const ScratchConvW&) = delete;
    ScratchConvW& operator=(const ScratchConvW&) = delete;
};

__global__ void op_scale_f64_kernel(double* buf, long long n, double f) {
    for (long long i = (long long)blockIdx.x * blockDim.x + threadIdx.x; i < n; i += (long long)gridDim.x * blockDim.x) buf[i] *= f;
}
int op_gbn_exchange(void* user, double* buf, long long count, void* stream) {
    long long blocks = (count + 255) / 256; if (blocks > 1024) blocks = 1024; if (blocks < 1) blocks = 1;
    hipLaunchKernelGGL(op_scale_f64_kernel, dim3((int)blocks), dim3(256), 0, (hipStream_t)stream, buf, count, (double)*(const int*)user);
    return hipGetLastError() == hipSuccess ? 0 : -5;
}
}

extern "C" {

int ptta_outlier_removal(const float* sparse, const float* validity, float* sparse_out, float* validity_out, int n, int height,
                         int width, int kernel_size, float threshold, float* scratch, ptta_stream s) {
    if (!sparse || !validity || !sparse_out || !validity_out || !scratch || n < 1 || height < 1 || width < 1 || kernel_size < 1 ||
        (kernel_size & 1) == 0) return -22;
    return ptta_launch_outlier_removal(sparse, validity, sparse_out, validity_out, n, height, width, kernel_size, threshold, scratch,
                                       (hipStream_t)s);
}

int ptta_eval_metrics(const float* depth, const float* ground_truth, int64_t numel, float min_evaluate_depth, float max_evaluate_depth,
                      void* scratch, float* metrics_out, ptta_stream s) {
    if (!depth || !ground_truth || !scratch || !metrics_out || numel < 1) return -22;
    return ptta_launch_eval_metrics(depth, ground_truth, numel, min_evaluate_depth, max_evaluate_depth, (double*)scratch, metrics_out,
                                    (hipStream_t)s);
}

static void dcn_args(DcnArgs& a, const float* input, const float* weight, const float* bias, const float* offset, const float* mask,
                     int b, int c, int h, int w, int c_out, int kh, int kw, int sh, int sw, int ph, int pw, int dh, int dw, int group, int dg) {
    a.in = input; a.weight = weight; a.bias = bias; a.offset = offset; a.mask = mask;
    a.B = b; a.C = c; a.H = h; a.W = w; a.Co = c_out; a.kh = kh; a.kw = kw; a.sh = sh; a.sw = sw; a.ph = ph; a.pw = pw;
    a.dh = dh; a.dw = dw; a.group = group; a.dg = dg;
}

int ptta_mdconv_forward(const float* input, const float* weight, const float* bias, const float* offset, const float* mask, float* output,
                        int b, int c, int h, int w, int c_out, int kh, int kw, int sh, int sw, int ph, int pw, int dh, int dw,
                        int group, int deformable_group, ptta_stream s) {
    if (!input || !weight || !offset || !mask || !output) return -22;
    DcnArgs a; dcn_args(a, input, weight, bias, offset, mask, b, c, h, w, c_out, kh, kw, sh, sw, ph, pw, dh, dw, group, deformable_group);
    a.out = output;
    return ptta_launch_dcn_forward(a, (hipStream_t)s);
}

int ptta_mdconv_backward(const float* input, const float* weight, const float* bias, const float* offset, const float* mask,
                         const float* grad_output, float* grad_input, float* grad_offset, float* grad_mask, float* grad_weight,
                         float* grad_bias, int b, int c, int h, int w, int c_out, int kh, int kw, int sh, int sw, int ph, int pw,
                         int dh, int dw, int group, int deformable_group, ptta_stream s) {
    if (!input || !weight || !offset || !mask || !grad_output) return -22;
    DcnArgs a; dcn_args(a, input, weight, bias, offset, mask, b, c, h, w, c_out, kh, kw, sh, sw, ph, pw, dh, dw, group, deformable_group);
    a.gout = grad_output; a.gin = grad_input; a.goff = grad_offset; a.gmask = grad_mask; a.gweight = grad_weight; a.gbias = grad_bias;
    return ptta_launch_dcn_backward(a, (hipStream_t)s);
}

int ptta_op_conv32(const float* in, const float* weight, const float* bias, float* out, int b, int hin, int win, int mode,
                   int relu_in, int in_major, int flip, int dtype, int naive, ptta_stream s_) {
    hipStream_t s = (hipStream_t)s_;
    ScratchConvW sw; ConvW& w = sw.w;
    void *tin = nullptr, *tout = nullptr;
    const int ho = mode == CONV_S1 ? hin : (mode == CONV_S2 ? hin / 2 : hin * 2), wo = mode == CONV_S1 ? win : (mode == CONV_S2 ? win / 2 : win * 2);
    const long nin = (long)b * hin * win * 32, nout = (long)b * ho * wo * 32;
    int rc = 0;
    if (!sw.ok || hipMalloc(&tin, nin * 2) != hipSuccess || hipMalloc(&tout, nout * 2) != hipSuccess) rc = -12;
    if (rc == 0) {
        ptta_pack_conv32(weight, w, in_major, flip, s);
        Conv32Args a; a.w = &w; a.bias = bias; a.B = b; a.Hin = hin; a.Win = win; a.mode = mode; a.relu_in = relu_in; a.naive = naive & 1; a.x3 = (naive >> 1) & 1;
        if (dtype != PTTA_DTYPE_F32) {
            from_f32_launch(in, (bf16_t*)tin, nin, s);
            a.in = tin; a.in_nb = b; a.out_raw = tout; a.bf16 = 1;
            rc = ptta_launch_conv32(a, s);
            to_f32_launch((const bf16_t*)tout, out, nout, s);
        } else {
            a.in = in; a.in_nb = b; a.out_raw = out; a.bf16 = 0;
            rc = ptta_launch_conv32(a, s);
        }
        (void)hipStreamSynchronize(s);
    }
    (void)hipFree(tin); (void)hipFree(tout);
    return rc;
}

int ptta_op_gwgrad(const float* x, const float* gy, float* gw, float* gb, int b, int h, int w, int ci, int co, int impl, int reps,
                   float* us_per_call_host, ptta_stream s_) {
    hipStream_t s = (hipStream_t)s_;
    if (!x || !gy || !gw || b < 1 || h < 1 || w < 1 || ci < 1 || co < 1 || ci > 256 || co > 256 || impl < 0 || impl > 2 || reps < 0 ||
        (reps > 0 && !us_per_call_host)) return -22;
    GView xv, gv;
    xv.p = (float*)x; xv.B = b; xv.H = h; xv.W = w; xv.C = ci; xv.ld = ci;
    gv.p = (float*)gy; gv.B = b; gv.H = h; gv.W = w; gv.C = co; gv.ld = co;
    const long P = (long)b * h * w;
    const size_t nm = (size_t)ptta_gwgrad_mfma_part_floats(P, ci, co), nn = (size_t)ptta_gwgrad_slabs(P) * (9 * ci * co + co);
    float* part = nullptr;
    if (hipMalloc((void**)&part, (impl == 2 ? nn : nm) * 4) != hipSuccess) return -12;
    auto run = [&]() {
        return impl == 0 ? ptta_launch_gwgrad_mfma(xv, gv, part, gw, gb, s)
                         : (impl == 1 ? ptta_launch_gwgrad_f32mfma(xv, gv, part, gw, gb, s) : ptta_launch_gwgrad(xv, gv, part, gw, gb, s));
    };
    int rc = run();
    if (!rc && reps > 0) {
        hipEvent_t e0 = nullptr, e1 = nullptr;
        if (hipEventCreate(&e0) != hipSuccess || hipEventCreate(&e1) != hipSuccess) rc = -5;
        if (!rc) {
            (void)hipEventRecord(e0, s);
            for (int r = 0; r < reps && !rc; ++r) rc = run();
            (void)hipEventRecord(e1, s);
            (void)hipEventSynchronize(e1);
            float ms = 0.f; (void)hipEventElapsedTime(&ms, e0, e1);
            *us_per_call_host = 1e3f * ms / (float)reps;
        }
        if (e0) (void)hipEventDestroy(e0);
        if (e1) (void)hipEventDestroy(e1);
    }
    if (hipStreamSynchronize(s) != hipSuccess && !rc) rc = -5;
    (void)hipFree(part);
    return rc;
}

int ptta_op_gconv(const float* x0, int c0, int ld0, const float* x1, int c1, int ld1, const float* weight, const float* bias, float* y, int co,
                  int ldy, int b, int hin, int win, int hout, int wout, int k, int geom, int act, int accumulate, int impl, int flags,
                  int six_b, int x1_from_b, int stat_npass, double* stat_host, int* form_host, ptta_stream s_) {
    hipStream_t s = (hipStream_t)s_;
    const bool vert = flags & PTTA_GCONV_VERT, dgrad = flags & PTTA_GCONV_DGRAD;
    if (!x0 || !weight || !y || b < 1 || hin < 1 || win < 1 || hout < 1 || wout < 1 || c0 < 1 || c1 < 0 || co < 1 || ld0 < c0 || ldy < co ||
        (c1 > 0) != (x1 != nullptr) || (c1 > 0 && ld1 < c1) || (k != 1 && k != 3) || geom < PTTA_GCONV_S1 || geom > PTTA_GCONV_T2 ||
        act < GACT_NONE || act > GACT_SIGMOID || impl < 0 || impl > 1 || (flags & ~7) || six_b < 0 || six_b > b || x1_from_b < 0 ||
        stat_npass < 0 || stat_npass > 2 || (accumulate & ~1)) return -22;
    if (vert && (k != 3 || geom != PTTA_GCONV_S1)) return -22;
    if (dgrad && (c1 > 0 || six_b > 0)) return -22;
    if (stat_npass > 0 && (!stat_host || geom != PTTA_GCONV_S1 || impl != 0 || dgrad || (b % stat_npass))) return -22;
    const int run = !dgrad ? geom : (geom == PTTA_GCONV_S2 ? PTTA_GCONV_T2 : (geom == PTTA_GCONV_T2 ? PTTA_GCONV_S2 : PTTA_GCONV_S1));
    const bool size_ok = run == PTTA_GCONV_S1 ? (hout == hin && wout == win)
                       : run == PTTA_GCONV_S2 ? (hout == (hin + 1) / 2 && wout == (win + 1) / 2)
                       : ((hout == 2 * hin || (dgrad && hout == 2 * hin - 1)) && (wout == 2 * win || (dgrad && wout == 2 * win - 1)));
    if (!size_ok) return -22;
    if (impl == 0 && ((((size_t)x0 | (size_t)x1) & 15) || (ld0 & 3) || (ld1 & 3))) return -22;
    if (form_host) *form_host = -1;

    gnet::GConvW cw;
    cw.k = k; cw.stride = geom == PTTA_GCONV_S1 ? 1 : 2; cw.transposed = geom == PTTA_GCONV_T2 ? 1 : 0; cw.vcol = vert ? 1 : 0;
    if (!dgrad) { cw.Ci = c0 + c1; cw.Co = co; cw.C0 = c0; cw.C1 = c1; }
    else { cw.Ci = co; cw.Co = c0; cw.C0 = co; cw.C1 = 0; }
    cw.mf = impl == 0 && !dgrad; cw.mb = impl == 0 && dgrad;
    const int KK = k * k;
    const size_t nw = (size_t)KK * cw.Ci * cw.Co;
    const size_t nfrag = cw.mf ? (size_t)ptta_gfrag_elems(KK, cw.C0, cw.C1, cw.Co) : (cw.mb ? (size_t)ptta_gfrag_elems(KK, cw.Co, 0, cw.Ci) : 0);
    const int tiles_pp = stat_npass ? ptta_gconv_x3_tiles(b / stat_npass, hout, wout) : 0;
    const size_t nstat = (size_t)stat_npass * tiles_pp * 2 * co;
    float* wbuf = nullptr; bf16_t* fbuf = nullptr; float* stat = nullptr;
    int rc = 0;
    if (hipMalloc((void**)&wbuf, 2 * nw * sizeof(float)) != hipSuccess || (nfrag && hipMalloc((void**)&fbuf, 3 * nfrag * sizeof(bf16_t)) != hipSuccess) ||
        (nstat && hipMalloc((void**)&stat, nstat * sizeof(float)) != hipSuccess)) rc = -12;
    if (!rc && (hipMemsetAsync(wbuf, 0, 2 * nw * sizeof(float), s) != hipSuccess || (nstat && hipMemsetAsync(stat, 0, nstat * sizeof(float), s) != hipSuccess))) rc = -5;
    if (!rc) {
        cw.wf = wbuf; cw.wb = wbuf + nw;
        if (cw.mf) { cw.ff_hi = fbuf; cw.ff_lo = fbuf + nfrag; if (six_b > 0) cw.ff_l2 = fbuf + 2 * nfrag; }
        if (cw.mb) { cw.fb_hi = fbuf; cw.fb_lo = fbuf + nfrag; }
        if (vert) gnet::pack_vcol_weight(cw, weight, s); else gnet::pack_conv_weight(cw, weight, s);
        GView xv[2], yv;
        xv[0].p = (float*)x0; xv[0].C = c0; xv[0].ld = ld0; xv[1].p = (float*)x1; xv[1].C = c1; xv[1].ld = ld1;
        for (GView& v : xv) { v.B = b; v.H = hin; v.W = win; }
        yv.p = y; yv.B = b; yv.H = hout; yv.W = wout; yv.C = co; yv.ld = ldy;
// ... 195 lines not shown
```

tta-depth-completion_amd/proxytta/_lib.py:

```python
import ctypes
import os
from ctypes import POINTER, byref, c_char_p, c_float, c_int, c_int64, c_uint64, c_void_p


_HERE = os.path.dirname(os.path.abspath(__file__))
LIB_PATH = os.path.join(_HERE, 'libptta_hip.so')

PTTA_BACKBONE_MSG_CHN = 0
PTTA_BACKBONE_NLSPN = 1
PTTA_BACKBONE_COSTDCNET = 2
PTTA_NLSPN_LEGACY_OFFSET = 0x100
PTTA_NLSPN_SYNCBN_ADAPT = 0x200
PTTA_SYNCBN_ADAPT = 0x200
PTTA_META_1LAYER = 0
PTTA_META_2LAYERS = 1
PTTA_DTYPE_F32 = 0
PTTA_DTYPE_MIXED = 1
PTTA_HEAD_FORM_PLAIN = 0
PTTA_HEAD_FORM_SYNCBN = 1
PTTA_ABI_VERSION = 2
CONV_S1, CONV_S2, CONV_T2 = 0, 1, 2


class Hparams(ctypes.Structure):
    _fields_ = [('lr', c_float), ('beta1', c_float), ('beta2', c_float), ('eps', c_float),
                ('weight_decay', c_float), ('w_sparse_depth', c_float), ('w_smoothness', c_float),
                ('w_cos', c_float), ('max_input_depth', c_float), ('max_predict_depth', c_float)]


class GbnView(ctypes.Structure):
    _fields_ = [('p', c_void_p), ('c', c_int), ('ld', c_int)]


class GbnArgs(ctypes.Structure):
    _fields_ = ([(n, c_int) for n in ('mode', 'b', 'h', 'w', 'npass', 'act', 'act_first', 'res_relu', 'acc_gx', 'acc_gres', 'world',
                                      'nblocks_in', 'repeats')] + [('eps', c_float), ('momentum', c_float)] +
                [(n, GbnView) for n in ('x', 'res', 'y', 'g', 'gx', 'gres')] +
                [(n, c_void_p) for n in ('gamma', 'beta', 'part_in', 'st', 'rm', 'rv', 'nbt', 'st_eval', 'dgamma', 'dbeta')])


_P = c_void_p
SIGNATURES = [
    ('ptta_create', c_int, [POINTER(c_void_p), c_int, c_int, c_int, c_int, c_int, c_int, POINTER(Hparams)]),
    ('ptta_destroy', None, [_P]),
    ('ptta_last_error', c_char_p, [_P]),
    ('ptta_set_hparams', c_int, [_P, POINTER(Hparams), _P]),
    ('ptta_load_weights', c_int, [_P, c_char_p, _P, POINTER(c_int64), c_int, _P]),
    ('ptta_bind_adapted', c_int, [_P, c_char_p, _P, _P, _P]),
    ('ptta_set_adam_step', c_int, [_P, c_int, _P]),
    ('ptta_get_adam_step', c_int, [_P, POINTER(c_int), _P]),
    ('ptta_forward_train', c_int, [_P, _P, _P, _P, _P, _P, _P]),
    ('ptta_embedding_rows', c_int64, [_P]),
    ('ptta_forward_eval', c_int, [_P, _P, _P, _P, _P]),
    ('ptta_loss_forward', c_int, [_P, _P, _P, _P, _P, _P, _P, c_int64, c_float, c_float, c_float, _P, _P]),
    ('ptta_loss_backward', c_int, [_P, _P, _P, _P, _P, _P, _P, c_int64, _P, _P, _P]),
    ('ptta_backward', c_int, [_P, _P, _P, _P, _P, _P]),
    ('ptta_set_grad', c_int, [_P, c_char_p, _P, c_int64, _P]),
    ('ptta_get_grad', c_int, [_P, c_char_p, _P, c_int64, _P]),
    ('ptta_adapted_count', c_int, [_P]),
    ('ptta_adapted_name', c_char_p, [_P, c_int, POINTER(c_int64)]),
    ('ptta_adapted_repeat', c_int, [_P, c_int]),
    ('ptta_adam_step', c_int, [_P, _P, _P, _P]),
    ('ptta_step', c_int, [_P, _P, _P, _P, _P, _P, _P, _P]),
    ('ptta_step_pipelined', c_int, [_P] * 5 + [c_uint64] + [_P] * 2 + [c_uint64] + [_P] * 3),
    ('ptta_pipeline_stream', c_int, [_P, POINTER(c_void_p)]),
    ('ptta_forward_eval_last', c_int, [_P, _P, _P]),
    ('ptta_outlier_removal', c_int, [_P, _P, _P, _P, c_int, c_int, c_int, c_int, c_float, _P, _P]),
    ('ptta_eval_metrics', c_int, [_P, _P, c_int64, c_float, c_float, _P, _P, _P]),
    ('ptta_mdconv_forward', c_int, [_P] * 6 + [c_int] * 15 + [_P]),
    ('ptta_mdconv_backward', c_int, [_P] * 11 + [c_int] * 15 + [_P]),
    ('ptta_set_image_norm', c_int, [_P, c_float, POINTER(c_float), POINTER(c_float)]),
    ('ptta_head_bind', c_int, [_P, c_char_p, _P, _P, _P]),
    ('ptta_head_set_hparams', c_int, [_P, c_float, c_float, c_float, c_float, c_float, c_float, c_int, _P]),
    ('ptta_head_reload', c_int, [_P, _P]),
    ('ptta_head_forward', c_int, [_P, _P, _P, c_int, _P, _P, _P]),
    ('ptta_head_backward', c_int, [_P, _P, _P]),
    ('ptta_head_adam_step', c_int, [_P, _P]),
    ('ptta_head_step', c_int, [_P, _P, _P, c_int, _P, _P]),
    ('ptta_head_get_grad', c_int, [_P, c_char_p, _P, c_int64, POINTER(c_int), _P]),
    ('ptta_head_set_form', c_int, [_P, c_int]),
    ('ptta_crop_flip', c_int, [_P, _P] + [c_int] * 6 + [_P] * 5),
    ('ptta_rotate', c_int, [_P, _P, c_int, c_int, c_int, c_int, _P, _P, c_int, _P]),
    ('ptta_resize_crop', c_int, [_P, _P, c_int, c_int, c_int, c_int, _P, _P, _P, _P, _P, c_int, c_int, _P]),
    ('ptta_photometric', c_int, [_P, _P, c_int, c_int, c_int, _P, _P, _P, _P, _P, _P, _P, _P]),
    ('ptta_photometric_full', c_int, [_P, _P, c_int, c_int, c_int] + [_P] * 12),
    ('ptta_add_noise', c_int, [_P, _P, _P, c_int, c_int, c_int, c_int, _P, c_float, c_int, _P]),
    ('ptta_remove_patches', c_int, [_P, _P, c_int, c_int, c_int, c_int, _P, _P, _P, _P, _P]),
    ('ptta_crop_pad', c_int, [_P, _P, c_int, c_int, c_int, c_int] + [_P] * 7 + [c_int, c_float, _P]),
    ('ptta_resize_pad', c_int, [_P, _P, c_int, c_int, c_int, c_int] + [_P] * 5 + [c_int, c_int, c_float, _P]),
    ('ptta_set_stat_sync', c_int, [_P, _P, _P, _P, c_int64, c_int]),
    ('ptta_rccl_unique_id', c_int, [_P]),
    ('ptta_rccl_comm_create', c_int, [_P, c_int, c_int, POINTER(c_void_p)]),
    ('ptta_rccl_comm_destroy', c_int, [_P]),
    ('ptta_rccl_allreduce_mean_f32', c_int, [_P, _P, c_int64, _P]),
    ('ptta_rccl_last_error', c_char_p, []),
    ('ptta_set_stat_sync_rccl', c_int, [_P, _P, _P, c_int64, c_int]),
    ('ptta_set_grad_sync_rccl', c_int, [_P, _P]),
    ('ptta_set_graph', c_int, [_P, c_int]),
    ('ptta_set_option', c_int, [_P, c_char_p, c_int]),
    ('ptta_get_option', c_int, [_P, c_char_p, POINTER(c_int)]),
    ('ptta_profile', c_int, [_P, c_int]),
    ('ptta_profile_read', c_int, [_P, c_int, POINTER(ctypes.c_double), POINTER(ctypes.c_double), POINTER(ctypes.c_double),
                                  POINTER(c_int64), _P]),
    ('ptta_debug_tensor', c_int, [_P, c_char_p, _P, c_int64, POINTER(c_int64), _P]),
    ('ptta_op_conv32', c_int, [_P, _P, _P, _P, c_int, c_int, c_int, c_int, c_int, c_int, c_int, c_int, c_int, _P]),
    ('ptta_op_conv32_chain', c_int, [_P] * 6 + [c_int] * 7 + [POINTER(c_float), _P]),
    ('ptta_op_gwgrad', c_int, [_P, _P, _P, _P] + [c_int] * 7 + [POINTER(c_float), _P]),
    ('ptta_op_gconv', c_int, [_P, c_int, c_int, _P, c_int, c_int, _P, _P, _P] + [c_int] * 16 + [POINTER(ctypes.c_double), POINTER(c_int), _P]),
    ('ptta_op_gbn', c_int, [POINTER(GbnArgs), _P]),
    ('ptta_version', c_int, []),
]

_lib = None


def load():
    global _lib
    if _lib is not None:
        return _lib
    import torch
    if not os.path.exists(LIB_PATH):
        raise RuntimeError('libptta_hip.so not found at %s: build it with `python -c "import '
                           '__graft_entry__ as g; g.build()"` — there is no CPU fallback' % LIB_PATH)
    lib = ctypes.CDLL(LIB_PATH)
    for name, res, args in SIGNATURES:
        fn = getattr(lib, name)
        fn.restype = res
        fn.argtypes = args
    have = lib.ptta_version()
    if have != PTTA_ABI_VERSION:
        raise RuntimeError('%s has ABI version %d, this binding is written against %d (include/ptta.h PTTA_ABI_VERSION): rebuild it with '
                           '`make -C tta-depth-completion_amd/csrc`' % (LIB_PATH, have, PTTA_ABI_VERSION))
    _lib = lib
    return lib


def check(lib, handle, rc, what):
    if rc != 0:
        msg = lib.ptta_last_error(handle).decode() if handle else ''
        raise RuntimeError('%s failed (%d): %s' % (what, rc, msg))


def ptr(t):
    if t is None:
        return None
    assert t.is_contiguous()
    return c_void_p(t.data_ptr())


__all__ = ['load', 'check', 'ptr', 'Hparams', 'GbnArgs', 'GbnView', 'SIGNATURES', 'LIB_PATH', 'byref']
```

tta-depth-completion_amd/proxytta/engine.py:

```python
import ctypes
from ctypes import byref, c_int, c_int64, c_void_p

import torch

from . import _lib
from ._lib import Hparams, check, ptr

ADAPTED = ('conv1_rgb_meta.weight', 'conv1_rgb_meta.bias')
_P2 = 'conv1_rgb_meta.conv1_meta.'
ADAPTED_2LAYERS = (_P2 + '0.0.weight', _P2 + '0.1.weight', _P2 + '0.1.bias', _P2 + '1.weight', _P2 + '1.bias',
                   _P2 + '2.weight', _P2 + '2.bias')


HEAD_PARAMS = tuple('%s.%s.%s' % (m, l, t) for m in ('proj', 'pred') for l in ('0', '1', '3') for t in ('weight', 'bias'))
HEAD_TARGETS = tuple('proj_t' + k[4:] for k in HEAD_PARAMS[:6])


def adapted_names(meta='1layer'):
    return ADAPTED_2LAYERS if meta == '2layers' else ADAPTED
_BOUND_SUFFIX = ('running_mean', 'running_var', 'num_batches_tracked')


def _stream():
    return c_void_p(torch.cuda.current_stream().cuda_stream)
# ... 325 lines not shown
        self._chk(self.lib.ptta_head_bind(self.handle, name.encode(), ptr(param), ptr(exp_avg), ptr(exp_avg_sq)), 'ptta_head_bind')
        self._fit_head_exchange()

    def set_head_hparams(self, lr=1e-3, betas=(0.9, 0.999), eps=1e-8, weight_decay=0.0, tau=0.999, adam_step=-1):
        self._chk(self.lib.ptta_head_set_hparams(self.handle, lr, betas[0], betas[1], eps, weight_decay, tau, int(adam_step), _stream()),
                  'ptta_head_set_hparams')

    def head_reload(self):
        self._chk(self.lib.ptta_head_reload(self.handle, _stream()), 'ptta_head_reload')

    def head_forward(self, image, sparse, reverse=True, want=True):
        image = self._f32(image, (self.n, 3, self.h, self.w))
        sparse = self._f32(sparse, (self.n, 1, self.h, self.w))
        emb = ref = None
        if want:
            emb = torch.empty((self.rows, self.emb_dim), device=image.device, dtype=torch.float32)
            ref = torch.empty_like(emb)
        self._chk(self.lib.ptta_head_forward(self.handle, ptr(image), ptr(sparse), int(bool(reverse)), ptr(emb), ptr(ref), _stream()),
                  'ptta_head_forward')
        return emb, ref

    def head_backward(self):
        loss = torch.empty(1, device=self.device, dtype=torch.float32)
        self._chk(self.lib.ptta_head_backward(self.handle, ptr(loss), _stream()), 'ptta_head_backward')
        return loss

    def head_adam_step(self):
        self._chk(self.lib.ptta_head_adam_step(self.handle, _stream()), 'ptta_head_adam_step')

    def head_step(self, image, sparse, reverse=True):
        image = self._f32(image, (self.n, 3, self.h, self.w))
        sparse = self._f32(sparse, (self.n, 1, self.h, self.w))
        loss = torch.empty(1, device=image.device, dtype=torch.float32)
        self._chk(self.lib.ptta_head_step(self.handle, ptr(image), ptr(sparse), int(bool(reverse)), ptr(loss), _stream()), 'ptta_head_step')
        return loss

    def head_grad(self, name, like):
        has = c_int(0)
        out = torch.empty_like(like)
        self._chk(self.lib.ptta_head_get_grad(self.handle, name.encode(), ptr(out), out.numel(), byref(has), _stream()), 'ptta_head_get_grad')
        return out if has.value else None

    def set_graph(self, enable):
        self._chk(self.lib.ptta_set_graph(self.handle, int(bool(enable))), 'ptta_set_graph')

    def set_option(self, key, value):
        self._chk(self.lib.ptta_set_option(self.handle, key.encode(), int(value)), 'ptta_set_option(%s)' % key)

    def get_option(self, key):
        v = ctypes.c_int(0)
        self._chk(self.lib.ptta_get_option(self.handle, key.encode(), byref(v)), 'ptta_get_option(%s)' % key)
        return v.value

    def profile(self, enable):
        self._chk(self.lib.ptta_profile(self.handle, int(bool(enable))), 'ptta_profile')

    def profile_read(self, klass):
        ms, by, mc, n = ctypes.c_double(0), ctypes.c_double(0), ctypes.c_double(0), c_int64(0)
        self._chk(self.lib.ptta_profile_read(self.handle, int(klass), byref(ms), byref(by), byref(mc), byref(n), _stream()),
                  'ptta_profile_read')
        return ms.value, by.value, mc.value, n.value

    def debug_tensor(self, name):
        n = c_int64(0)
        self._chk(self.lib.ptta_debug_tensor(self.handle, name.encode(), None, 0, byref(n), _stream()), 'ptta_debug_tensor')
        out = torch.empty(n.value, device=self.device, dtype=torch.float32)
        self._chk(self.lib.ptta_debug_tensor(self.handle, name.encode(), ptr(out), n.value, byref(n), _stream()),
                  'ptta_debug_tensor')
        return out


def op_conv32(x_nhwc, weight, bias, mode, relu_in=False, in_major=False, flip=False, dtype='fp32', naive=False, x3=False):
    lib = _lib.load()
    b, h, w, _ = x_nhwc.shape
    ho, wo = {0: (h, w), 1: (h // 2, w // 2), 2: (2 * h, 2 * w)}[mode]
    out = torch.empty((b, ho, wo, 32), device=x_nhwc.device, dtype=torch.float32)
    rc = lib.ptta_op_conv32(ptr(x_nhwc.contiguous()), ptr(weight.contiguous()), ptr(bias), ptr(out), b, h, w, mode,
                            int(relu_in), int(in_major), int(flip), 0 if dtype == 'fp32' else 1, int(bool(naive)) | (2 if x3 else 0), _stream())
    if rc != 0:
        raise RuntimeError('ptta_op_conv32 failed (%d)' % rc)
    return out


GWGRAD_IMPLS = {'default': 0, 'fp32_mfma': 1, 'naive': 2}


def op_gwgrad(x_nhwc, gy_nhwc, impl='default', with_bias=True, reps=0):
    lib = _lib.load()
    b, h, w, ci = x_nhwc.shape
    co = gy_nhwc.shape[3]
    assert tuple(gy_nhwc.shape[:3]) == (b, h, w)
    x_nhwc, gy_nhwc = x_nhwc.float().contiguous(), gy_nhwc.float().contiguous()
    gw = torch.empty((co, ci, 3, 3), device=x_nhwc.device, dtype=torch.float32)
    gb = torch.empty((co,), device=x_nhwc.device, dtype=torch.float32) if with_bias else None
    us = ctypes.c_float(0.0)
    rc = lib.ptta_op_gwgrad(ptr(x_nhwc), ptr(gy_nhwc), ptr(gw), ptr(gb), b, h, w, ci, co,
                            GWGRAD_IMPLS[impl], int(reps), byref(us), _stream())
    if rc != 0:
        raise RuntimeError('ptta_op_gwgrad failed (%d)' % rc)
    return gw, gb, (us.value if reps > 0 else None)


GCONV_GEOMS = {'s1': 0, 's2': 1, 't2': 2}
GCONV_ACTS = {'none': 0, 'relu': 1, 'lrelu': 2, 'sigmoid': 3}
GCONV_IMPLS = {'mfma': 0, 'direct': 1}
GCONV_FORMS = {-1: None, 0: 'plain', 1: 'nco2', 2: 'ksplit'}


def op_gconv(x0, weight, y, x1=None, bias=None, k=3, geom='s1', act='none', accumulate=False, impl='mfma', vert=False, six_b=0,
             x1_from_b=None, x1_w2=False, dgrad=False, stat_npass=0):
    lib = _lib.load()

    def view(t):
        b, h, w, c = t.shape
        ld = t.stride(2)
        assert t.dtype == torch.float32 and t.stride(3) == 1 and t.stride(1) == w * ld and t.stride(0) == h * w * ld and ld >= c
        return c_void_p(t.data_ptr()), c, ld
    b, hin, win, _ = x0.shape
    hout, wout = y.shape[1], y.shape[2]
    assert y.shape[0] == b and (x1 is None or tuple(x1.shape[:3]) == (b, hin, win))
    p0, c0, ld0 = view(x0)
    p1, c1, ld1 = view(x1) if x1 is not None else (None, 0, 0)
    py, co, ldy = view(y)
    stats = (ctypes.c_double * (stat_npass * 2 * co))() if stat_npass else None
    form = c_int(-1)
    flags = (1 if vert else 0) | (2 if x1_w2 else 0) | (4 if dgrad else 0)
    rc = lib.ptta_op_gconv(p0, c0, ld0, p1, c1, ld1, ptr(weight.contiguous()), ptr(bias), py, co, ldy, b, hin, win, hout, wout, k,
                           GCONV_GEOMS[geom], GCONV_ACTS[act], int(bool(accumulate)), GCONV_IMPLS[impl], flags, int(six_b),
                           (1 << 30) if x1_from_b is None else int(x1_from_b), int(stat_npass), stats, byref(form), _stream())
    if rc != 0:
        raise RuntimeError('ptta_op_gconv failed (%d)' % rc)
    st = torch.tensor(list(stats), dtype=torch.float64).view(stat_npass, 2, co) if stat_npass else None
    return GCONV_FORMS[form.value], st


GBN_MODES = {'train': 0, 'eval': 1, 'backward': 2}
GBN_ACTS = {'none': 0, 'relu': 1, 'lrelu': 2, 'elu': 4}


def op_gbn(mode, x, y, st, gamma, beta=None, res=None, g=None, gx=None, gres=None, npass=1, act='none', act_first=False, res_relu=True,
           acc_gx=False, acc_gres=False, eps=1e-5, part_in=None, rm=None, rv=None, nbt=None, momentum=0.1, repeats=1, st_eval=None,
           dgamma=None, dbeta=None, world=1):
    lib = _lib.load()
    b, h, w, _ = x.shape
    a = _lib.GbnArgs()

    def view(t, images):
        if t is None:
            return _lib.GbnView(None, 0, 0)
        n, hh, ww, c = t.shape
        ld = t.stride(2)
        assert t.dtype == torch.float32 and (n, hh, ww) == (images, h, w), 'views disagree in size'
        assert t.stride(3) == 1 and t.stride(1) == w * ld and t.stride(0) == h * w * ld
        return _lib.GbnView(t.data_ptr(), c, ld)

    def table(t, dtype=torch.float32):
        if t is None:
            return None
        assert t.dtype == dtype and t.is_contiguous()
        return t.data_ptr()
    per = b // npass if mode == 'backward' else b
    a.mode, a.b, a.h, a.w, a.npass = GBN_MODES[mode], b, h, w, int(npass)
    a.act, a.act_first, a.res_relu, a.acc_gx, a.acc_gres = GBN_ACTS[act], int(bool(act_first)), int(bool(res_relu)), int(bool(acc_gx)), int(bool(acc_gres))
    a.world, a.repeats, a.eps, a.momentum = int(world), int(repeats), float(eps), float(momentum)
    a.nblocks_in = int(part_in.shape[1]) if part_in is not None else 0
    a.x, a.y, a.res = view(x, b), view(y, b), view(res, b)
# ... 8 lines not shown
```

Measured before the change: 814.1.

## Fuse stride-2/transposed conv32 with following stride-1 conv into one kernel

Adds a pair kernel that computes a strided or transposed 3x3 conv over a tile plus its halo, keeps the intermediate activation in LDS, and immediately applies the following stride-1 conv with its epilogue. It is used for the encoder and decoder conv pairs in the MSG-CHN forward pass when the launch is small (tile count at most 256). The aim is to cut one launch and the global round trip of the intermediate in low-occupancy regimes. In exchange, halo recomputation and heavy register and LDS use limit the kernel to one block per CU, and the kernel still writes the raw intermediate out.

```diff
diff --git a/include/ptta.h b/include/ptta.h
--- a/include/ptta.h
+++ b/include/ptta.h
@@ -152,6 +152,10 @@
 int ptta_op_conv32(const float* in_nhwc, const float* weight, const float* bias, float* out_nhwc,
                    int b, int hin, int win, int mode, int relu_in, int in_major, int flip, int dtype, int naive,
                    ptta_stream s);
+int ptta_op_conv32_pair(const float* in_nhwc, const float* weight1, const float* bias1, const float* weight2, const float* bias2,
+                        const float* add1_first, const float* add1_second, float* mid_nhwc, float* out_nhwc,
+                        int b, int hin, int win, int mode1, int relu2, int in_nb, int dtype, int fused, int* fused_used_host,
+                        ptta_stream s);
 int ptta_op_gwgrad(const float* x_nhwc, const float* gy_nhwc, float* gw, float* gb, int b, int h, int w, int ci, int co, int impl,
                    int reps, float* us_per_call_host, ptta_stream s);
 #define PTTA_GCONV_S1 0
diff --git a/tta-depth-completion_amd/csrc/conv32.hip b/tta-depth-completion_amd/csrc/conv32.hip
--- a/tta-depth-completion_amd/csrc/conv32.hip
+++ b/tta-depth-completion_amd/csrc/conv32.hip
@@ -1053,6 +1053,254 @@
     }
 }
 
+#define PF_RH 6
+#define PF_RW 34
+template <typename T, int MODE, bool UP, bool ADD>
+__global__ __launch_bounds__(256, 1) void conv32_pair_kernel(Conv32P<T> p1, Conv32P<T> p2) {
+    constexpr bool F32 = sizeof(T) == 4;
+    constexpr bool S2 = MODE == CONV_S2;
+    constexpr int STR = Geo<T>::STR;
+    constexpr int UPH = 4, UPW = 18;
+    constexpr int WSTR = S2 ? (F32 ? S2_STR : 48) : STR;
+    constexpr int WPH = S2 ? 2 * PF_RH + 1 : 4, WPW = S2 ? 2 * PF_RW + 1 : 18;
+    constexpr int WNPIX = WPH * WPW;
+    constexpr int MID = PF_RH * PF_RW * STR, WIN = WNPIX * WSTR, WL1 = F32 ? 18 * 64 * 16 : 0;
+    constexpr int NITEM = S2 ? 2 : 3;
+    __shared__ __attribute__((aligned(16))) unsigned char lds[MID + WIN + WL1 + (UP ? UPH * UPW * Geo<T>::UPPX : 0)];
+    unsigned char* const win = lds + MID;
+    unsigned char* const wl1_lds = win + WIN;
+    unsigned char* const up_lds = wl1_lds + WL1;
+    const int tid = threadIdx.x, lane = tid & 63;
+    const int i = lane & 31, h = lane >> 5;
+    const float bias1 = epi_bias(p1.epi, i), bias2 = epi_bias(p2.epi, i);
+    const int wave = __builtin_amdgcn_readfirstlane(tid >> 6);
+    const int H = p2.Hout, W = p2.Wout, Hin = p1.Hin, Win = p1.Win;
+    const int ntx = (W + 31) >> 5, nty = (H + X3S_TH - 1) / X3S_TH;
+    const float sy = up_scale(H >> 1, H), sx = up_scale(W >> 1, W);
+    const int tile = blockIdx.x;
+    const int ty_ = tile % nty, tx_ = (tile / nty) % ntx, b = tile / (nty * ntx);
+    const int y0 = ty_ * X3S_TH, x0 = tx_ << 5;
+    const int wy0 = S2 ? 2 * y0 - 3 : (y0 >> 1) - 1, wx0 = S2 ? 2 * x0 - 3 : (x0 >> 1) - 1;
+    constexpr int NIT = (WNPIX * 4 + 255) / 256;
+    const T* inb = p1.in + (size_t)(b % p1.in_nb) * Hin * Win * 32;
+    Px<T> v[NIT];
+    bool vok[NIT];
+#pragma unroll
+    for (int it = 0; it < NIT; ++it) {
+        const int idx = tid + 256 * it;
+        const int g = idx & 3, pix = idx >> 2;
+        const int py = pix / WPW, px = pix - py * WPW;
+        const int gy = wy0 + py, gx = wx0 + px;
+        vok[it] = pix < WNPIX && gy >= 0 && gy < Hin && gx >= 0 && gx < Win;
+        v[it] = px_load(inb + ((size_t)min(max(gy, 0), Hin - 1) * Win + min(max(gx, 0), Win - 1)) * 32 + 8 * g);
+    }
+    uint4 wh1[9][2], wh2[9][2], wl2[F32 ? 9 : 1][2];
+    constexpr int NWL = F32 ? (18 * 64 + 255) / 256 : 1;
+    uint4 wl1_t[NWL];
+    {
+        const uint4* ph = (const uint4*)p1.wpack;
+#pragma unroll
+        for (int t = 0; t < 9; ++t)
+#pragma unroll
+            for (int k = 0; k < 2; ++k) wh1[t][k] = ph[(t * 2 + k) * 64 + lane];
+        if constexpr (F32) {
+            const uint4* pl = (const uint4*)p1.wpack2;
+#pragma unroll
+            for (int k = 0; k < NWL; ++k) wl1_t[k] = pl[min(tid + 256 * k, 18 * 64 - 1)];
+        }
+        const uint4* ph2 = (const uint4*)p2.wpack;
+#pragma unroll
+        for (int t = 0; t < 9; ++t)
+#pragma unroll
+            for (int k = 0; k < 2; ++k) wh2[t][k] = ph2[(t * 2 + k) * 64 + lane];
+        if constexpr (F32) {
+            const uint4* pl2 = (const uint4*)p2.wpack2;
+#pragma unroll
+            for (int t = 0; t < 9; ++t)
+#pragma unroll
+                for (int k = 0; k < 2; ++k) wl2[t][k] = pl2[(t * 2 + k) * 64 + lane];
+        }
+    }
+    int uy0 = 0, ux0 = 0;
+    constexpr int NUP = UP ? (UPH * UPW * Geo<T>::UPPC + 255) / 256 : 1;
+    uint4 upv[NUP];
+    if (UP) {
+        const int Hu = H >> 1, Wu = W >> 1;
+        uy0 = lerp_coef(y0, Hu, sy).i0; ux0 = lerp_coef(x0, Wu, sx).i0;
+        const T* ub = p2.epi.up + (size_t)(b % p2.epi.up_nb) * Hu * Wu * 32;
+        constexpr int PC = Geo<T>::UPPC;
+#pragma unroll
+        for (int k = 0; k < NUP; ++k) {
+            const int idx = min(tid + 256 * k, UPH * UPW * PC - 1);
+            const int q = idx % PC, pix = idx / PC;
+            const int r = pix / UPW, cc = pix - r * UPW;
+            const int gy = min(uy0 + r, Hu - 1), gx = min(ux0 + cc, Wu - 1);
+            upv[k] = *(const uint4*)(ub + ((size_t)gy * Wu + gx) * 32 + (32 / PC) * q);
+        }
+    }
+#pragma unroll
+    for (int it = 0; it < NIT; ++it) if (!vok[it]) v[it] = px_zero<T>();
+    if constexpr (F32) {
+#pragma unroll
+        for (int k = 0; k < NWL; ++k) if (tid + 256 * k < 18 * 64) *(uint4*)(wl1_lds + (tid + 256 * k) * 16) = wl1_t[k];
+    }
+    f32x16 acc[NITEM];
+#pragma unroll
+    for (int n = 0; n < NITEM; ++n)
+#pragma unroll
+        for (int r = 0; r < 16; ++r) acc[n][r] = 0.f;
+    if constexpr (S2) {
+        const int gq = (tid >> 1) & 1;
+#pragma unroll
+        for (int q = 0; q < 2; ++q) {
+            if (q == 1) lds_barrier();
+            if (gq == q) {
+#pragma unroll
+                for (int it = 0; it < NIT; ++it) {
+                    const int idx = tid + 256 * it;
+                    const int pix = idx >> 2;
+                    if (pix < WNPIX) px_stage<true>(v[it], win + pix * WSTR + 16 * (idx & 1), 32);
+                }
+            }
+            lds_barrier();
+#pragma unroll
+            for (int n = 0; n < NITEM; ++n) {
+                const int item = wave + 4 * n;
+                if (item < 7) {
+                    const int r = item < 6 ? item : min(i >> 1, PF_RH - 1);
+                    const int cc = item < 6 ? i + 1 : ((i & 1) ? PF_RW - 1 : 0);
+#pragma unroll
+                    for (int tap = 0; tap < 9; ++tap) {
+                        const int ky = tap / 3, kx = tap % 3;
+                        const unsigned char* a = win + ((2 * r + ky) * WPW + 2 * cc + kx) * WSTR + 16 * h;
+                        const bf16x8 ah = __builtin_bit_cast(bf16x8, *(const uint4*)a);
+                        const bf16x8 bh = __builtin_bit_cast(bf16x8, wh1[tap][q]);
+                        if constexpr (F32) {
+                            const bf16x8 al = __builtin_bit_cast(bf16x8, *(const uint4*)(a + 32));
+                            const bf16x8 bl = __builtin_bit_cast(bf16x8, *(const uint4*)(wl1_lds + ((tap * 2 + q) * 64 + lane) * 16));
+                            acc[n] = __builtin_amdgcn_mfma_f32_32x32x16_bf16(al, bh, acc[n], 0, 0, 0);
+                            acc[n] = __builtin_amdgcn_mfma_f32_32x32x16_bf16(ah, bl, acc[n], 0, 0, 0);
+                        }
+                        acc[n] = __builtin_amdgcn_mfma_f32_32x32x16_bf16(ah, bh, acc[n], 0, 0, 0);
+                    }
+                }
+            }
+        }
+    } else {
+#pragma unroll
+        for (int it = 0; it < NIT; ++it) {
+            const int idx = tid + 256 * it;
+            const int pix = idx >> 2;
+            if (pix < WNPIX) px_stage<true>(v[it], win + pix * WSTR + 16 * (idx & 3), Geo<T>::LO);
+        }
+        lds_barrier();
+#pragma unroll
+        for (int n = 0; n < NITEM; ++n) {
+            const int item = wave + 4 * n;
+            const int r = item >> 1, par = item & 1;
+            const int y = y0 - 1 + r;
+            const int x = i < 16 ? x0 + par + 2 * i : (i == 16 ? (par ? x0 - 1 : x0 + 32) : x0 + par);
+#pragma unroll
+            for (int tap = 0; tap < 9; ++tap) {
+                const int ky = tap / 3, kx = tap % 3;
+                const int ty = y + 1 - ky;
+                const int yi = ty >> 1;
+                if ((ty & 1) == 0 && ((par + 1 - kx) & 1) == 0 && yi >= 0 && yi < Hin) {
+                    const int xi = (x + 1 - kx) >> 1;
+                    const unsigned char* a = win + ((yi - wy0) * WPW + (xi - wx0)) * WSTR + 16 * h;
+#pragma unroll
+                    for (int k = 0; k < 2; ++k) {
+                        const bf16x8 ah = __builtin_bit_cast(bf16x8, *(const uint4*)(a + 32 * k));
+                        const bf16x8 bh = __builtin_bit_cast(bf16x8, wh1[tap][k]);
+                        if constexpr (F32) {
+                            const bf16x8 al = __builtin_bit_cast(bf16x8, *(const uint4*)(a + 32 * k + 64));
+                            const bf16x8 bl = __builtin_bit_cast(bf16x8, *(const uint4*)(wl1_lds + ((tap * 2 + k) * 64 + lane) * 16));
+                            acc[n] = __builtin_amdgcn_mfma_f32_32x32x16_bf16(al, bh, acc[n], 0, 0, 0);
+                            acc[n] = __builtin_amdgcn_mfma_f32_32x32x16_bf16(ah, bl, acc[n], 0, 0, 0);
+                        }
+                        acc[n] = __builtin_amdgcn_mfma_f32_32x32x16_bf16(ah, bh, acc[n], 0, 0, 0);
+                    }
+                }
+            }
+        }
+    }
+#pragma unroll
+    for (int n = 0; n < NITEM; ++n) {
+        const int item = wave + 4 * n;
+        if (S2 && item >= 7) continue;
+        const int rr = S2 ? item : item >> 1, par = item & 1;
+        const int y = y0 - 1 + rr;
+        if ((!S2 || item < 6) && rr >= 1 && rr <= X3S_TH && y < H) {
+            if constexpr (S2) epi_tile<T, false, false, false>(p1.epi, b, y, H, W, i, acc[n], x0, h, W, 1, 0, 0.f, 0.f, nullptr, 0, 0, &bias1);
+            else epi_tile<T, false, false, false>(p1.epi, b, y, H, W, i, acc[n], x0 >> 1, h, min(Win, (x0 >> 1) + 16), 2, par, 0.f, 0.f, nullptr, 0, 0, &bias1);
+        }
+        f32x16 t;
+#pragma unroll
+        for (int r = 0; r < 16; ++r) t[r] = acc[n][r] + bias1;
+        quad_transpose(t, lane);
+        const int j4 = (i >> 2) * 4;
+#pragma unroll
+        for (int g = 0; g < 4; ++g) {
+            const int m = (i & 3) + 8 * g + 4 * h;
+            int r, cc;
+            bool have;
+            if constexpr (S2) {
+                if (item < 6) { r = item; cc = m + 1; have = true; }
+                else { r = m >> 1; cc = (m & 1) ? PF_RW - 1 : 0; have = m < 2 * PF_RH; }
+            } else {
+                r = rr; cc = m < 16 ? 1 + par + 2 * m : (par ? 0 : PF_RW - 1); have = m <= 16;
+            }
+            if (!have) continue;
+            const int yy = y0 - 1 + r, xx = x0 - 1 + cc;
+            const bool inside = yy >= 0 && yy < H && xx >= 0 && xx < W;
+            float4 val = make_float4(t[4 * g], t[4 * g + 1], t[4 * g + 2], t[4 * g + 3]);
+            if (!inside) val = make_float4(0.f, 0.f, 0.f, 0.f);
+            unsigned char* dst = lds + (r * PF_RW + cc) * STR + 2 * j4;
+            if constexpr (F32) {
+                val = relu4(val);
+                uint2 hi, lo;
+                split2(val.x, val.y, hi.x, lo.x); split2(val.z, val.w, hi.y, lo.y);
+                *(uint2*)dst = hi;
+                *(uint2*)(dst + Geo<T>::LO) = lo;
+            } else {
+                uint2 hb = f4_to_bf4(val);
+                hb.x = relu_pk(hb.x); hb.y = relu_pk(hb.y);
+                *(uint2*)dst = hb;
+            }
+        }
+    }
+    if (UP) {
+#pragma unroll
+        for (int k = 0; k < NUP; ++k) if (tid + 256 * k < UPH * UPW * Geo<T>::UPPC) *(uint4*)(up_lds + (size_t)(tid + 256 * k) * 16) = upv[k];
+    }
+    lds_barrier();
+    const int y = y0 + wave;
+    if (y < H) {
+        f32x16 acc2;
+#pragma unroll
+        for (int r = 0; r < 16; ++r) acc2[r] = 0.f;
+#pragma unroll
+        for (int tap = 0; tap < 9; ++tap) {
+            const int ky = tap / 3, kx = tap % 3;
+            const unsigned char* a = lds + ((wave + ky) * X3_PW + i + kx) * STR + 16 * h;
+#pragma unroll
+            for (int k = 0; k < 2; ++k) {
+                const bf16x8 ah = __builtin_bit_cast(bf16x8, *(const uint4*)(a + 32 * k));
+                const bf16x8 bh = __builtin_bit_cast(bf16x8, wh2[tap][k]);
+                if constexpr (F32) {
+                    const bf16x8 al = __builtin_bit_cast(bf16x8, *(const uint4*)(a + 32 * k + 64));
+                    const bf16x8 bl = __builtin_bit_cast(bf16x8, wl2[tap][k]);
+                    acc2 = __builtin_amdgcn_mfma_f32_32x32x16_bf16(al, bh, acc2, 0, 0, 0);
+                    acc2 = __builtin_amdgcn_mfma_f32_32x32x16_bf16(ah, bl, acc2, 0, 0, 0);
+                }
+                acc2 = __builtin_amdgcn_mfma_f32_32x32x16_bf16(ah, bh, acc2, 0, 0, 0);
+            }
+        }
+        if (UP) epi_tile<T, false, false, ADD, true, UPW>(p2.epi, b, y, H, W, i, acc2, x0, h, W, 1, 0, sy, sx, up_lds, uy0, ux0, &bias2);
+        else epi_tile<T, false, false, ADD>(p2.epi, b, y, H, W, i, acc2, x0, h, W, 1, 0, sy, sx, nullptr, 0, 0, &bias2);
+    }
+}
+
 template <typename T, int MODE, bool RELU>
 __global__ void conv32_naive_kernel(Conv32P<T> p) {
     const long total = (long)p.B * p.Hout * p.Wout * 32;
@@ -1316,6 +1564,53 @@
     return a.bf16 ? launch_first_t<bf16_t>(a, f, a_out, a_nb, bwd_form, tiles, s) : launch_first_t<float>(a, f, a_out, a_nb, bwd_form, tiles, s);
 }
 
+template <typename T, int MODE>
+static int launch_pair_t(const Conv32Args& a1, const Conv32Args& a2, hipStream_t s) {
+    auto fill = [](Conv32P<T>& p, const Conv32Args& a, int Ho, int Wo) {
+        p.in = (const T*)a.in; p.in_nb = a.in_nb > 0 ? a.in_nb : 1;
+        p.wpack = a.w->mbf16; p.wpack2 = sizeof(T) == 4 ? a.w->mlo : nullptr;
+        p.epi.bias = a.bias;
+        p.epi.up = (const T*)a.up; p.epi.up_nb = a.up_nb > 0 ? a.up_nb : 1;
+        p.epi.mask = nullptr; p.epi.mask_nb = 1;
+        p.epi.add1 = (const T*)a.add1; p.epi.add1_nb = a.add1_nb > 0 ? a.add1_nb : 1;
+        p.epi.add2 = (const T*)a.add2; p.epi.add2_nb = a.add2_nb > 0 ? a.add2_nb : 1;
+        p.epi.out_raw = (T*)a.out_raw; p.epi.out_sum = (T*)a.out_sum;
+        p.epi.mask_bits = nullptr; p.epi.bits_out = a.bits_out; p.epi.bits_nb = a.bits_nb; p.epi.bits_sum = a.bits_sum;
+        p.B = a.B; p.Hin = a.Hin; p.Win = a.Win; p.Hout = Ho; p.Wout = Wo;
+    };
+    Conv32P<T> p1, p2;
+    fill(p1, a1, a2.Hin, a2.Win);
+    fill(p2, a2, a2.Hin, a2.Win);
+    const int blocks = a2.B * ((a2.Win + 31) / 32) * ((a2.Hin + X3S_TH - 1) / X3S_TH);
+#define KP_(U, A) hipLaunchKernelGGL((conv32_pair_kernel<T, MODE, U, A>), dim3(blocks), dim3(256), 0, s, p1, p2)
+    if constexpr (MODE == CONV_S2) {
+        if (a2.up) { if (a2.add1) KP_(true, true); else KP_(true, false); }
+        else { if (a2.add1) KP_(false, true); else KP_(false, false); }
+    } else {
+        if (a2.add1) KP_(false, true); else KP_(false, false);
+    }
+#undef KP_
+    PTTA_CHECK_LAUNCH();
+    return 0;
+}
+bool ptta_conv32_pair_applies(const Conv32Args& a1, const Conv32Args& a2) { return ptta_launch_conv32_pair(a1, a2, nullptr, true) == 0; }
+int ptta_launch_conv32_pair(const Conv32Args& a1, const Conv32Args& a2, hipStream_t s, bool check_only) {
+    if (a1.mode != CONV_S2 && a1.mode != CONV_T2) return 1;
+    if (!a1.w || !a2.w || !a1.in) return 1;
+    if (a2.mode != CONV_S1 || a1.bf16 != a2.bf16 || a1.naive || a2.naive || a1.w2 || a2.w2) return 1;
+    if (!a1.bf16 && (!a1.x3 || !a2.x3)) return 1;
+    if (!a1.relu_in || a1.up || a1.mask || a1.add1 || a1.add2 || a1.out_sum || !a1.out_raw || a1.mask_bits) return 1;
+    if (!a2.relu_in || a2.mask || a2.mask_bits || (a2.add2 && !a2.add1) || (a2.up && a1.mode == CONV_T2)) return 1;
+    if (a1.bf16 && (a1.bits_out || a2.bits_out)) return 1;
+    const int Ho = a1.mode == CONV_S2 ? a1.Hin / 2 : a1.Hin * 2, Wo = a1.mode == CONV_S2 ? a1.Win / 2 : a1.Win * 2;
+    if (a2.in != a1.out_raw || a2.in_nb != a2.B || a1.B != a2.B || a2.Hin != Ho || a2.Win != Wo || Ho < 1 || Wo < 1) return 1;
+    const long tiles8 = (long)a2.B * ((Wo + 31) / 32) * ((Ho + X3_TH - 1) / X3_TH);
+    if (tiles8 > 256) return 1;
+    if (check_only) return 0;
+    if (a1.bf16) return a1.mode == CONV_S2 ? launch_pair_t<bf16_t, CONV_S2>(a1, a2, s) : launch_pair_t<bf16_t, CONV_T2>(a1, a2, s);
+    return a1.mode == CONV_S2 ? launch_pair_t<float, CONV_S2>(a1, a2, s) : launch_pair_t<float, CONV_T2>(a1, a2, s);
+}
+
 int ptta_launch_conv32(const Conv32Args& a, hipStream_t s) {
     if (a.bf16) {
         if (a.mode == CONV_S1) return launch_conv32_t<bf16_t, CONV_S1>(a, s);
diff --git a/tta-depth-completion_amd/csrc/msgchn_ctx.h b/tta-depth-completion_amd/csrc/msgchn_ctx.h
--- a/tta-depth-completion_amd/csrc/msgchn_ctx.h
+++ b/tta-depth-completion_amd/csrc/msgchn_ctx.h
@@ -117,6 +117,7 @@
     hipEvent_t ev_loss = nullptr;
     hipEvent_t ev_dpart = nullptr;
     int fuse_first = 1, fuse_head_bwd = 1;
+    int fuse_pair = 1;
     int cos_grad_fused = 1;
     bool cos_in_gemm = false;
     void* w0frag = nullptr; float *hm_part = nullptr, *headP = nullptr; double* head_k12 = nullptr;
@@ -282,6 +283,8 @@
 int conv_out1_p(ptta_ctx* c, const ConvOut1Args& a, hipStream_t s);
 int conv32(ptta_ctx* c, hipStream_t s, const std::string& layer, bool bwd, int mode, const void* in, int in_nb,
            int B, int Hin, int Win, bool relu, const E& e);
+int conv32_pair(ptta_ctx* c, hipStream_t s, const std::string& l1, int mode1, const void* in, int in_nb, int B, int Hin, int Win,
+                const E& e1, const std::string& l2, const E& e2);
 int conv32w(ptta_ctx* c, hipStream_t s, const ConvW* w, const float* bias, const void* in, int in_nb, int B, int H, int W, const E& e);
 int conv32_first_bwd(ptta_ctx* c, hipStream_t s, const std::string& layer, ConvInArgs& f, int B, int H, int W, const E& e);
 int to_narrow(ptta_ctx* c, const void* src_f32, void* dst, long n, hipStream_t s);
diff --git a/tta-depth-completion_amd/csrc/msgchn_forward.hip b/tta-depth-completion_amd/csrc/msgchn_forward.hip
--- a/tta-depth-completion_amd/csrc/msgchn_forward.hip
+++ b/tta-depth-completion_amd/csrc/msgchn_forward.hip
@@ -20,11 +20,10 @@
     return ptta_launch_conv_out1(a, s);
 }
 
-int conv32(ptta_ctx* c, hipStream_t s, const std::string& layer, bool bwd, int mode, const void* in, int in_nb,
-           int B, int Hin, int Win, bool relu, const E& e) {
+static int conv32_args(ptta_ctx* c, const std::string& layer, bool bwd, int mode, const void* in, int in_nb,
+                       int B, int Hin, int Win, bool relu, const E& e, Conv32Args& a, int& es_l_out) {
     auto it = c->l32.find(layer);
     if (it == c->l32.end()) return c->fail("unknown 32->32 layer " + layer, -2);
-    Conv32Args a;
     a.in = in; a.in_nb = in_nb; a.w = bwd ? &it->second.b : &it->second.f;
     a.bias = bwd ? nullptr : (layer == "conv1_rgb_meta" ? c->meta_b : it->second.bias);
     a.up = e.up; a.up_nb = e.up_nb; a.mask = e.mask; a.mask_nb = e.mask_nb;
@@ -42,6 +41,15 @@
             if (bs || br) { a.bits_out = bs ? bs : br; a.bits_sum = bs ? 1 : 0; a.bits_nb = c->Nn; }
         }
     }
+    es_l_out = es_l;
+    return 0;
+}
+
+int conv32(ptta_ctx* c, hipStream_t s, const std::string& layer, bool bwd, int mode, const void* in, int in_nb,
+           int B, int Hin, int Win, bool relu, const E& e) {
+    Conv32Args a;
+    int es_l = 4;
+    { const int rc = conv32_args(c, layer, bwd, mode, in, in_nb, B, Hin, Win, relu, e, a, es_l); if (rc) return rc; }
     const long pin = (long)B * Hin * Win;
     const long pout = mode == CONV_S1 ? pin : (mode == CONV_S2 ? pin / 4 : pin * 4);
     const bool small = (long)Hin * Win <= (long)c->H4 * c->W4 * (mode == CONV_S2 ? 4 : 1);
@@ -51,6 +59,26 @@
     ProfScope ps(c, (mode == CONV_S1 ? (relu ? 0 : 2) : 4) + (small ? 1 : 0), s, (double)((pin + pout) * 32 + 9216) * es_l,
                  (double)(mode == CONV_T2 ? pin : pout) * 9.0 * 32.0 * 32.0, 1);
     return ptta_launch_conv32(a, s);
+}
+
+int conv32_pair(ptta_ctx* c, hipStream_t s, const std::string& l1, int mode1, const void* in, int in_nb, int B, int Hin, int Win,
+                const E& e1, const std::string& l2, const E& e2) {
+    const int Ho = mode1 == CONV_S2 ? Hin / 2 : Hin * 2, Wo = mode1 == CONV_S2 ? Win / 2 : Win * 2;
+    if (c->fuse_pair && !c->naive && (c->x3 || c->bf16 || e1.nar) && e1.nar == e2.nar) {
+        Conv32Args a1, a2;
+        int es1 = 4, es2 = 4;
+        { const int rc = conv32_args(c, l1, false, mode1, in, in_nb, B, Hin, Win, true, e1, a1, es1); if (rc) return rc; }
+        { const int rc = conv32_args(c, l2, false, CONV_S1, e1.raw, B, B, Ho, Wo, true, e2, a2, es2); if (rc) return rc; }
+        if (ptta_conv32_pair_applies(a1, a2)) {
+            const long pin = (long)B * Hin * Win, pmid = (long)B * Ho * Wo;
+            ProfScope ps(c, 5, s, (double)((pin + pmid) * 32 + 9216) * es1 + (double)(2 * pmid * 32 + 9216) * es2,
+                         (double)((mode1 == CONV_T2 ? pin : pmid) + pmid) * 9.0 * 32.0 * 32.0, 1);
+            const int rc = ptta_launch_conv32_pair(a1, a2, s);
+            return rc == 1 ? c->fail("conv32_pair: fused form refused a case its caller accepted", -22) : rc;
+        }
+    }
+    { const int rc = conv32(c, s, l1, false, mode1, in, in_nb, B, Hin, Win, true, e1); if (rc) return rc; }
+    return conv32(c, s, l2, false, CONV_S1, e1.raw, B, B, Ho, Wo, true, e2);
 }
 
 int conv32w(ptta_ctx* c, hipStream_t s, const ConvW* w, const float* bias, const void* in, int in_nb, int B, int H, int W, const E& e) {
@@ -234,14 +262,10 @@
         a.B = nb; a.H = H1; a.W = W1; a.bf16 = c->bf16; a.naive = c->naive;
         RUN(conv32_first(c, s, "rgb_encoder.init.2", a, 0, nb, H1, W1, e_raw(at(c->c0, H1, W1))));
     }
-    CV("rgb_encoder.enc1.1", false, CONV_S2, at(c->c0, H1, W1), nb, nb, H1, W1, true, e_raw(at(c->c1a, H2, W2)));
-    CV("rgb_encoder.enc1.3", false, CONV_S1, at(c->c1a, H2, W2), nb, nb, H2, W2, true, e_raw(at(c->c1, H2, W2)));
-    CV("rgb_encoder.enc2.1", false, CONV_S2, at(c->c1, H2, W2), nb, nb, H2, W2, true, e_raw(at(c->c2a, H4, W4)));
-    CV("rgb_encoder.enc2.3", false, CONV_S1, at(c->c2a, H4, W4), nb, nb, H4, W4, true, e_raw(at(c->c2, H4, W4)));
-    CV("rgb_encoder.enc3.1", false, CONV_S2, at(c->c2, H4, W4), nb, nb, H4, W4, true, e_raw(at(c->c3a, H8, W8)));
-    CV("rgb_encoder.enc3.3", false, CONV_S1, at(c->c3a, H8, W8), nb, nb, H8, W8, true, e_raw(at(c->c3, H8, W8)));
-    CV("rgb_encoder.enc4.1", false, CONV_S2, at(c->c3, H8, W8), nb, nb, H8, W8, true, e_raw(at(c->c4a, H16, W16)));
-    CV("rgb_encoder.enc4.3", false, CONV_S1, at(c->c4a, H16, W16), nb, nb, H16, W16, true, e_raw(at(c->c4, H16, W16)));
+    RUN(conv32_pair(c, s, "rgb_encoder.enc1.1", CONV_S2, at(c->c0, H1, W1), nb, nb, H1, W1, e_raw(at(c->c1a, H2, W2)), "rgb_encoder.enc1.3", e_raw(at(c->c1, H2, W2))));
+    RUN(conv32_pair(c, s, "rgb_encoder.enc2.1", CONV_S2, at(c->c1, H2, W2), nb, nb, H2, W2, e_raw(at(c->c2a, H4, W4)), "rgb_encoder.enc2.3", e_raw(at(c->c2, H4, W4))));
+    RUN(conv32_pair(c, s, "rgb_encoder.enc3.1", CONV_S2, at(c->c2, H4, W4), nb, nb, H4, W4, e_raw(at(c->c3a, H8, W8)), "rgb_encoder.enc3.3", e_raw(at(c->c3, H8, W8))));
+    RUN(conv32_pair(c, s, "rgb_encoder.enc4.1", CONV_S2, at(c->c3, H8, W8), nb, nb, H8, W8, e_raw(at(c->c4a, H16, W16)), "rgb_encoder.enc4.3", e_raw(at(c->c4, H16, W16))));
     return 0;
 }
 
@@ -289,12 +313,16 @@
     const int Bf = two ? Nn : B2;
     { E e; e.raw = c->e1_1; e.sum = c->y1; e.add1 = c->c3; e.add1_nb = B2;
       RUN(conv32(c, s, "depth_encoder1.enc1.3", false, CONV_S1, c->e1_1a, Nn, Bf, H8, W8, true, e)); }
-    { E e; e.raw = c->e1_2a; RUN(conv32(c, s, "depth_encoder1.enc2.1", false, CONV_S2, c->e1_1, B2, Nn, H8, W8, true, e)); }
-    { E e; e.sum = c->y2; e.add1 = c->c4; e.add1_nb = B2;
-      RUN(conv32(c, s, "depth_encoder1.enc2.3", false, CONV_S1, c->e1_2a, Nn, Bf, H16, W16, true, e)); }
-    { E e; e.raw = c->t1; RUN(conv32(c, s, "depth_decoder1.dec2.1", false, CONV_T2, c->y2, B2, Bf, H16, W16, true, e)); }
-    { E e; e.raw = c->y3; e.sum = c->s1_1; e.add1 = c->y1; e.add1_nb = B2;
-      RUN(conv32(c, s, "depth_decoder1.dec2.3", false, CONV_S1, c->t1, B2, Bf, H8, W8, true, e)); }
+    { E e1; e1.raw = c->e1_2a;
+      E e; e.sum = c->y2; e.add1 = c->c4; e.add1_nb = B2;
+      if (Bf == Nn) RUN(conv32_pair(c, s, "depth_encoder1.enc2.1", CONV_S2, c->e1_1, B2, Nn, H8, W8, e1, "depth_encoder1.enc2.3", e));
+      else {
+          RUN(conv32(c, s, "depth_encoder1.enc2.1", false, CONV_S2, c->e1_1, B2, Nn, H8, W8, true, e1));
+          RUN(conv32(c, s, "depth_encoder1.enc2.3", false, CONV_S1, c->e1_2a, Nn, Bf, H16, W16, true, e));
+      } }
+    { E e1; e1.raw = c->t1;
+      E e; e.raw = c->y3; e.sum = c->s1_1; e.add1 = c->y1; e.add1_nb = B2;
+      RUN(conv32_pair(c, s, "depth_decoder1.dec2.1", CONV_T2, c->y2, B2, Bf, H16, W16, e1, "depth_decoder1.dec2.3", e)); }
     { E e; e.raw = c->u1; RUN(conv32(c, s, "depth_decoder1.dec1.1", false, CONV_T2, c->s1_1, B2, Bf, H8, W8, true, e)); }
     if (!two) return 0;
     RUN(to_narrow(c, c->e1_0, c->tw(c->e1_0), (long)Nn * H4 * W4 * 32, s));
@@ -304,9 +332,9 @@
       RUN(conv32(c, s, "depth_encoder1.enc1.3", false, CONV_S1, c->tw(c->e1_1a), Nn, Nn, H8, W8, true, e)); }
     { E e; e.nar = true; e.sum = c->tw(c->y2); e.add1 = c->tw(c->c4); e.add1_nb = Nn;
       RUN(conv32(c, s, "depth_encoder1.enc2.3", false, CONV_S1, c->tw(c->e1_2a), Nn, Nn, H16, W16, true, e)); }
-    { E e; e.nar = true; e.raw = c->tw(c->t1); RUN(conv32(c, s, "depth_decoder1.dec2.1", false, CONV_T2, c->tw(c->y2), Nn, Nn, H16, W16, true, e)); }
-    { E e; e.nar = true; e.raw = c->tw(c->y3); e.sum = c->tw(c->s1_1); e.add1 = c->tw(c->y1); e.add1_nb = Nn;
-      RUN(conv32(c, s, "depth_decoder1.dec2.3", false, CONV_S1, c->tw(c->t1), Nn, Nn, H8, W8, true, e)); }
+    { E e1; e1.nar = true; e1.raw = c->tw(c->t1);
+      E e; e.nar = true; e.raw = c->tw(c->y3); e.sum = c->tw(c->s1_1); e.add1 = c->tw(c->y1); e.add1_nb = Nn;
+      RUN(conv32_pair(c, s, "depth_decoder1.dec2.1", CONV_T2, c->tw(c->y2), Nn, Nn, H16, W16, e1, "depth_decoder1.dec2.3", e)); }
     { E e; e.nar = true; e.raw = c->tw(c->u1); RUN(conv32(c, s, "depth_decoder1.dec1.1", false, CONV_T2, c->tw(c->s1_1), Nn, Nn, H8, W8, true, e)); }
     return 0;
 }
@@ -327,6 +355,7 @@
         auto raw = [&](void* r) { E e; e.raw = r; e.nar = nar; return e; };
         const void* e1_0 = nar ? c->tw(c->e1_0) : c->e1_0;
 #define CR(...) RUN(conv32(c, st, __VA_ARGS__))
+#define CP(...) RUN(conv32_pair(c, st, __VA_ARGS__))
         { E e; e.nar = nar; e.raw = A(c->y4, H4, W4); e.sum = A(c->s0_1, H4, W4); e.add1 = e1_0; e.add1_nb = Nn; e.add2 = A(c->m, H4, W4); e.add2_nb = Bl;
           CR("depth_decoder1.dec1.3", false, CONV_S1, A(c->u1, H4, W4), Bl, Bl, H4, W4, true, e); }
         CR("depth_decoder1.prdct.1", false, CONV_S1, A(c->s0_1, H4, W4), Bl, Bl, H4, W4, true, raw(A(c->v1, H4, W4)));
@@ -347,17 +376,14 @@
             E e; e.nar = nar; e.raw = A(c->e2_0, H2, W2); e.up = A(c->y4, H4, W4); e.up_nb = Bl;
             RUN(conv32_first(c, st, "depth_encoder2.init.2", a, (b0 == 0 && !nar) ? Nn : 0, Bl, H2, W2, e));
         }
-        CR("depth_encoder2.enc1.1", false, CONV_S2, A(c->e2_0, H2, W2), Bl, Bl, H2, W2, true, raw(A(c->e2_1a, H4, W4)));
-        { E e; e.nar = nar; e.raw = A(c->e2_1, H4, W4); e.up = A(c->y3, H8, W8); e.up_nb = Bl; CR("depth_encoder2.enc1.3", false, CONV_S1, A(c->e2_1a, H4, W4), Bl, Bl, H4, W4, true, e); }
-        CR("depth_encoder2.enc2.1", false, CONV_S2, A(c->e2_1, H4, W4), Bl, Bl, H4, W4, true, raw(A(c->e2_2a, H8, W8)));
+        { E e; e.nar = nar; e.raw = A(c->e2_1, H4, W4); e.up = A(c->y3, H8, W8); e.up_nb = Bl;
+          CP("depth_encoder2.enc1.1", CONV_S2, A(c->e2_0, H2, W2), Bl, Bl, H2, W2, raw(A(c->e2_1a, H4, W4)), "depth_encoder2.enc1.3", e); }
         { E e; e.nar = nar; e.sum = A(c->z2, H8, W8); e.up = A(c->y2, H16, W16); e.up_nb = Bl; e.add1 = A(c->c3, H8, W8); e.add1_nb = Bl;
-          CR("depth_encoder2.enc2.3", false, CONV_S1, A(c->e2_2a, H8, W8), Bl, Bl, H8, W8, true, e); }
-        CR("depth_decoder2.dec2.1", false, CONV_T2, A(c->z2, H8, W8), Bl, Bl, H8, W8, true, raw(A(c->t2, H4, W4)));
+          CP("depth_encoder2.enc2.1", CONV_S2, A(c->e2_1, H4, W4), Bl, Bl, H4, W4, raw(A(c->e2_2a, H8, W8)), "depth_encoder2.enc2.3", e); }
         { E e; e.nar = nar; e.raw = A(c->z3, H4, W4); e.sum = A(c->s1_2, H4, W4); e.add1 = A(c->e2_1, H4, W4); e.add1_nb = Bl; e.add2 = A(c->m, H4, W4); e.add2_nb = Bl;
-          CR("depth_decoder2.dec2.3", false, CONV_S1, A(c->t2, H4, W4), Bl, Bl, H4, W4, true, e); }
-        CR("depth_decoder2.dec1.1", false, CONV_T2, A(c->s1_2, H4, W4), Bl, Bl, H4, W4, true, raw(A(c->u2, H2, W2)));
+          CP("depth_decoder2.dec2.1", CONV_T2, A(c->z2, H8, W8), Bl, Bl, H8, W8, raw(A(c->t2, H4, W4)), "depth_decoder2.dec2.3", e); }
         { E e; e.nar = nar; e.raw = A(c->z4, H2, W2); e.sum = A(c->s0_2, H2, W2); e.add1 = A(c->e2_0, H2, W2); e.add1_nb = Bl; e.add2 = A(c->c1, H2, W2); e.add2_nb = Bl;
-          CR("depth_decoder2.dec1.3", false, CONV_S1, A(c->u2, H2, W2), Bl, Bl, H2, W2, true, e); }
+          CP("depth_decoder2.dec1.1", CONV_T2, A(c->s1_2, H4, W4), Bl, Bl, H4, W4, raw(A(c->u2, H2, W2)), "depth_decoder2.dec1.3", e); }
         CR("depth_decoder2.prdct.1", false, CONV_S1, A(c->s0_2, H2, W2), Bl, Bl, H2, W2, true, raw(A(c->v2, H2, W2)));
         {
             const LOut& lo = c->lout["depth_decoder2.prdct.3"];
@@ -376,13 +402,13 @@
             E e; e.nar = nar; e.raw = A(c->e3_0, H1, W1); e.up = A(c->z4, H2, W2); e.up_nb = Bl;
             RUN(conv32_first(c, st, "depth_encoder3.init.2", a, (b0 == 0 && !nar) ? Nn : 0, Bl, H1, W1, e));
         }
-        CR("depth_encoder3.enc1.1", false, CONV_S2, A(c->e3_0, H1, W1), Bl, Bl, H1, W1, true, raw(A(c->e3_1a, H2, W2)));
-        { E e; e.nar = nar; e.raw = A(c->e3_1, H2, W2); e.up = A(c->z3, H4, W4); e.up_nb = Bl; CR("depth_encoder3.enc1.3", false, CONV_S1, A(c->e3_1a, H2, W2), Bl, Bl, H2, W2, true, e); }
-        CR("depth_encoder3.enc2.1", false, CONV_S2, A(c->e3_1, H2, W2), Bl, Bl, H2, W2, true, raw(A(c->e3_2a, H4, W4)));
+        { E e; e.nar = nar; e.raw = A(c->e3_1, H2, W2); e.up = A(c->z3, H4, W4); e.up_nb = Bl;
+          CP("depth_encoder3.enc1.1", CONV_S2, A(c->e3_0, H1, W1), Bl, Bl, H1, W1, raw(A(c->e3_1a, H2, W2)), "depth_encoder3.enc1.3", e); }
         { E e; e.nar = nar; e.raw = A(c->feat, H4, W4); e.up = A(c->z2, H8, W8); e.up_nb = Bl; e.add1 = A(c->m, H4, W4); e.add1_nb = Bl;
           if (!nar) e.sum = A(c->w2, H4, W4); else e.add1 = nullptr;
-          CR("depth_encoder3.enc2.3", false, CONV_S1, A(c->e3_2a, H4, W4), Bl, Bl, H4, W4, true, e); }
+          CP("depth_encoder3.enc2.1", CONV_S2, A(c->e3_1, H2, W2), Bl, Bl, H2, W2, raw(A(c->e3_2a, H4, W4)), "depth_encoder3.enc2.3", e); }
 #undef CR
+#undef CP
         return 0;
     };
     if (two) {
@@ -416,12 +442,10 @@
         }
     }
     if (!c->skip_dec3) {
-    CV("depth_decoder3.dec2.1", false, CONV_T2, c->w2, B2, Nn, H4, W4, true, e_raw(c->t3));
     { E e; e.sum = c->s1_3; e.add1 = c->e3_1; e.add1_nb = B2; e.add2 = c->c1; e.add2_nb = B2;
-      CV("depth_decoder3.dec2.3", false, CONV_S1, c->t3, Nn, Nn, H2, W2, true, e); }
-    CV("depth_decoder3.dec1.1", false, CONV_T2, c->s1_3, Nn, Nn, H2, W2, true, e_raw(c->u3));
+      RUN(conv32_pair(c, s, "depth_decoder3.dec2.1", CONV_T2, c->w2, B2, Nn, H4, W4, e_raw(c->t3), "depth_decoder3.dec2.3", e)); }
     { E e; e.sum = c->s0_3; e.add1 = c->e3_0; e.add1_nb = B2; e.add2 = c->c0; e.add2_nb = B2;
-      CV("depth_decoder3.dec1.3", false, CONV_S1, c->u3, Nn, Nn, H1, W1, true, e); }
+      RUN(conv32_pair(c, s, "depth_decoder3.dec1.1", CONV_T2, c->s1_3, Nn, Nn, H2, W2, e_raw(c->u3), "depth_decoder3.dec1.3", e)); }
     CV("depth_decoder3.prdct.1", false, CONV_S1, c->s0_3, Nn, Nn, H1, W1, true, e_raw(c->v3));
     {
         const LOut& lo = c->lout["depth_decoder3.prdct.3"];
diff --git a/tta-depth-completion_amd/csrc/ptta_api.hip b/tta-depth-completion_amd/csrc/ptta_api.hip
--- a/tta-depth-completion_amd/csrc/ptta_api.hip
+++ b/tta-depth-completion_amd/csrc/ptta_api.hip
@@ -386,7 +386,7 @@
     {"fuse_first", &ptta_ctx::fuse_first, 2, false},    {"fuse_head_bwd", &ptta_ctx::fuse_head_bwd, 1, false},
     {"fuse_heads", &ptta_ctx::fuse_heads, 1, false},    {"heads_v2", &ptta_ctx::heads_v2, 1, false},
     {"cos_in_gemm", &ptta_ctx::cos_grad_fused, 1, false}, {"mask_bits", &ptta_ctx::mask_bits_on, 1, false},
-    {"stamps", &ptta_ctx::stamps, 1, true},
+    {"stamps", &ptta_ctx::stamps, 1, true},               {"fuse_pair", &ptta_ctx::fuse_pair, 1, true},
 };
 static const Option* find_option(const std::string& k) {
     for (const Option& o : kOptions) if (k == o.key) return &o;
diff --git a/tta-depth-completion_amd/csrc/ptta_kernels.h b/tta-depth-completion_amd/csrc/ptta_kernels.h
--- a/tta-depth-completion_amd/csrc/ptta_kernels.h
+++ b/tta-depth-completion_amd/csrc/ptta_kernels.h
@@ -37,6 +37,8 @@
 };
 void ptta_pack_conv32(const float* src, const ConvW& w, int in_major, int flip, hipStream_t s, int row_stride = 32, int col_off = 0);
 int ptta_launch_conv32(const Conv32Args& a, hipStream_t s);
+int ptta_launch_conv32_pair(const Conv32Args& a1, const Conv32Args& a2, hipStream_t s, bool check_only = false);
+bool ptta_conv32_pair_applies(const Conv32Args& a1, const Conv32Args& a2);
 int ptta_launch_conv32_loop(const Conv32Args& a, void* buf_a, void* buf_b, int reps, unsigned* ctr, unsigned* base_io, int* err, int variant, hipStream_t s);
 
 struct Plane { const float* p = nullptr; int nb = 1; long bstride = 0;
diff --git a/tta-depth-completion_amd/csrc/ptta_ops.hip b/tta-depth-completion_amd/csrc/ptta_ops.hip
--- a/tta-depth-completion_amd/csrc/ptta_ops.hip
+++ b/tta-depth-completion_amd/csrc/ptta_ops.hip
@@ -93,6 +93,55 @@
         (void)hipStreamSynchronize(s);
     }
     (void)hipFree(tin); (void)hipFree(tout);
+    return rc;
+}
+
+int ptta_op_conv32_pair(const float* in, const float* weight1, const float* bias1, const float* weight2, const float* bias2,
+                        const float* add1_first, const float* add1_second, float* mid, float* out, int b, int hin, int win, int mode1,
+                        int relu2, int in_nb, int dtype, int fused, int* fused_used_host, ptta_stream s_) {
+    hipStream_t s = (hipStream_t)s_;
+    if (!in || !weight1 || !weight2 || !mid || !out || b < 1 || hin < 1 || win < 1 || in_nb < 1 || in_nb > b ||
+        (mode1 != CONV_S2 && mode1 != CONV_T2)) return -22;
+    ScratchConvW sw1, sw2;
+    const int ho = mode1 == CONV_S2 ? hin / 2 : hin * 2, wo = mode1 == CONV_S2 ? win / 2 : win * 2;
+    if (ho < 1 || wo < 1) return -22;
+    const long nin = (long)in_nb * hin * win * 32, nout = (long)b * ho * wo * 32;
+    const bool nar = dtype != PTTA_DTYPE_F32;
+    void* t[5] = {nullptr, nullptr, nullptr, nullptr, nullptr};
+    int rc = (sw1.ok && sw2.ok) ? 0 : -12, used = 0;
+    if (rc == 0 && nar) {
+        const long n[5] = {nin, add1_first ? nout : 0, add1_second ? nout : 0, nout, nout};
+        for (int k = 0; k < 5 && rc == 0; ++k) if (n[k] && hipMalloc(&t[k], n[k] * 2) != hipSuccess) rc = -12;
+    }
+    if (rc == 0) {
+        ptta_pack_conv32(weight1, sw1.w, mode1 == CONV_T2 ? 1 : 0, 0, s);
+        ptta_pack_conv32(weight2, sw2.w, 0, 0, s);
+        if (nar) {
+            from_f32_launch(in, (bf16_t*)t[0], nin, s);
+            if (add1_first) from_f32_launch(add1_first, (bf16_t*)t[1], nout, s);
+            if (add1_second) from_f32_launch(add1_second, (bf16_t*)t[2], nout, s);
+        }
+        Conv32Args a1, a2;
+        a1.w = &sw1.w; a1.bias = bias1; a1.B = b; a1.Hin = hin; a1.Win = win; a1.mode = mode1; a1.relu_in = 1; a1.x3 = 1; a1.bf16 = nar ? 1 : 0;
+        a1.in = nar ? t[0] : (const void*)in; a1.in_nb = in_nb;
+        void* const midp = nar ? t[3] : (void*)mid;
+        if (add1_first) { a1.add1 = nar ? t[1] : (const void*)add1_first; a1.add1_nb = b; a1.out_sum = midp; }
+        else a1.out_raw = midp;
+        a2.w = &sw2.w; a2.bias = bias2; a2.B = b; a2.Hin = ho; a2.Win = wo; a2.mode = CONV_S1; a2.relu_in = relu2 ? 1 : 0; a2.x3 = 1; a2.bf16 = a1.bf16;
+        a2.in = midp; a2.in_nb = b; a2.out_raw = nar ? t[4] : (void*)out;
+        if (add1_second) {
+            a2.add1 = nar ? t[2] : (const void*)add1_second; a2.add1_nb = b; a2.out_sum = a2.out_raw; a2.out_raw = nullptr;
+        }
+        if (fused) {
+            rc = ptta_launch_conv32_pair(a1, a2, s);
+            if (rc == 0) used = 1; else if (rc == 1) rc = 0;
+        }
+        if (rc == 0 && !used) { rc = ptta_launch_conv32(a1, s); if (rc == 0) rc = ptta_launch_conv32(a2, s); }
+        if (rc == 0 && nar) { to_f32_launch((const bf16_t*)t[3], mid, nout, s); to_f32_launch((const bf16_t*)t[4], out, nout, s); }
+        if (hipStreamSynchronize(s) != hipSuccess && rc == 0) rc = -5;
+    }
+    for (void* q : t) (void)hipFree(q);
+    if (fused_used_host) *fused_used_host = used;
     return rc;
 }
 
diff --git a/tta-depth-completion_amd/proxytta/_lib.py b/tta-depth-completion_amd/proxytta/_lib.py
--- a/tta-depth-completion_amd/proxytta/_lib.py
+++ b/tta-depth-completion_amd/proxytta/_lib.py
@@ -105,6 +105,7 @@
     ('ptta_debug_tensor', c_int, [_P, c_char_p, _P, c_int64, POINTER(c_int64), _P]),
     ('ptta_op_conv32', c_int, [_P, _P, _P, _P, c_int, c_int, c_int, c_int, c_int, c_int, c_int, c_int, c_int, _P]),
     ('ptta_op_conv32_chain', c_int, [_P] * 6 + [c_int] * 7 + [POINTER(c_float), _P]),
+    ('ptta_op_conv32_pair', c_int, [_P] * 9 + [c_int] * 8 + [POINTER(c_int), _P]),
     ('ptta_op_gwgrad', c_int, [_P, _P, _P, _P] + [c_int] * 7 + [POINTER(c_float), _P]),
     ('ptta_op_gconv', c_int, [_P, c_int, c_int, _P, c_int, c_int, _P, _P, _P] + [c_int] * 16 + [POINTER(ctypes.c_double), POINTER(c_int), _P]),
     ('ptta_op_gbn', c_int, [POINTER(GbnArgs), _P]),
diff --git a/tta-depth-completion_amd/proxytta/engine.py b/tta-depth-completion_amd/proxytta/engine.py
--- a/tta-depth-completion_amd/proxytta/engine.py
+++ b/tta-depth-completion_amd/proxytta/engine.py
@@ -431,6 +431,23 @@
     return out
 
 
+def op_conv32_pair(x_nhwc, weight1, bias1, weight2, bias2, mode1, b=None, relu2=True, add1_first=None, add1_second=None, dtype='fp32',
+                   fused=True):
+    lib = _lib.load()
+    in_nb, h, w, _ = x_nhwc.shape
+    b = in_nb if b is None else b
+    ho, wo = {1: (h // 2, w // 2), 2: (2 * h, 2 * w)}[mode1]
+    mid = torch.empty((b, ho, wo, 32), device=x_nhwc.device, dtype=torch.float32)
+    out = torch.empty_like(mid)
+    used = ctypes.c_int(0)
+    keep = [t.contiguous() if t is not None else None for t in (x_nhwc, weight1, bias1, weight2, bias2, add1_first, add1_second)]
+    rc = lib.ptta_op_conv32_pair(*[ptr(t) for t in keep], ptr(mid), ptr(out), b, h, w, mode1, int(relu2), in_nb,
+                                 0 if dtype == 'fp32' else 1, int(fused), byref(used), _stream())
+    if rc != 0:
+        raise RuntimeError('ptta_op_conv32_pair failed (%d)' % rc)
+    return mid, out, bool(used.value)
+
+
 GWGRAD_IMPLS = {'default': 0, 'fp32_mfma': 1, 'naive': 2}
 
 
```

After: 784.1. 0.963x the previous value.
